# ChanghyeonKim93/visual_odometry_ros

Measured on AMD Instinct MI355X. Metric: stereo VO frames/sec @1241x376, 1500 feats, higher is better.
Workload: dtype u8/i32 (KLT, FAST) + f32 (IC, GN, DLT) + f64 (local BA)

## Files before the change

include/vo_hip.h:

```cpp
#ifndef VO_HIP_H_
#define VO_HIP_H_

#include <stddef.h>
#include <stdint.h>

#ifdef __cplusplus
extern "C" {
#endif

#define VO_HIP_ABI_VERSION 3

typedef enum {
  VO_OK = 0,
  VO_ERR_INVALID = -1,
  VO_ERR_HIP = -2,
  VO_ERR_NO_DEVICE = -3,
  VO_ERR_SIZE = -4,
  VO_ERR_NAN_AXAY = -5,
  VO_ERR_NAN_PATCH = -6,
  VO_ERR_NAN_UPDATE = -7,
  VO_ERR_CAPACITY = -8,
  VO_ERR_GN_FAILED = -9,
  VO_ERR_LBA_NAN = -10
} vo_status;

#define VO_KLT_USE_INITIAL_FLOW 4

#define VO_GN_VARIANT_CORE 0
#define VO_GN_VARIANT_STANDALONE 1

typedef struct vo_ctx vo_ctx;

typedef struct {
  int device;
  int max_width;
  int max_height;
  int max_points;
  int n_slots;
  int max_level;
} vo_config;

typedef struct {
  int iterations;
  float err;
  float delta_err;
  float delta_norm;
  int cnt_invalid;
  int is_nan;
} vo_gn_info;

int vo_abi_version(void);
int vo_device_count(void);
int vo_create(const vo_config *cfg, vo_ctx **out);
void vo_destroy(vo_ctx *ctx);
const char *vo_last_error(const vo_ctx *ctx);
void *vo_stream(vo_ctx *ctx);
int vo_synchronize(vo_ctx *ctx);

enum { VO_SUM_ORDER_TREE = 0, VO_SUM_ORDER_REFERENCE = 1 };
int vo_set_sum_order(vo_ctx *ctx, int order);
int vo_get_sum_order(const vo_ctx *ctx);

int vo_set_image(vo_ctx *ctx, int slot, const uint8_t *host, int width, int height, int stride);
int vo_set_image_device(vo_ctx *ctx, int slot, const void *dev, int width, int height, int stride);
int vo_swap_slots(vo_ctx *ctx, int slot_a, int slot_b);
int vo_set_stereo_pair_device(vo_ctx *ctx, int slot_l, const void *dev_l, int slot_r, const void *dev_r,
                              int width, int height, int stride);
int vo_set_ingest_side_stream(vo_ctx *ctx, int on);
int vo_set_stereo_pair_host_async(vo_ctx *ctx, int slot_l, const uint8_t *host_l, int slot_r, const uint8_t *host_r,
                                  int width, int height, int stride);
int vo_set_pyramid_window_hint(vo_ctx *ctx, int win);
int vo_pyramid_levels(int width, int height, int win, int max_level);
int vo_get_level(vo_ctx *ctx, int slot, int level, uint8_t *host, int *width, int *height);

int vo_klt_track(vo_ctx *ctx, int slot0, int slot1, const float *pts0, float *pts1, int n,
                 int win, int max_level, int flags, int max_iter, double eps, float min_eig_thr,
                 uint8_t *status, float *err);

int vo_track(vo_ctx *ctx, int slot0, int slot1, const float *pts0, int n, int win, int max_level,
             float thres_err, float *pts_track, uint8_t *mask_valid);
int vo_track_bidirection(vo_ctx *ctx, int slot0, int slot1, const float *pts0, int n, int win,
                         int max_level, float thres_err, float thres_bidirection,
                         float *pts_track, uint8_t *mask_valid);
int vo_track_bidirection_with_prior(vo_ctx *ctx, int slot0, int slot1, const float *pts0, int n,
                                    int win, int max_level, float thres_err,
                                    float thres_bidirection, float *pts_track,
                                    uint8_t *mask_valid);
int vo_track_with_prior(vo_ctx *ctx, int slot0, int slot1, const float *pts0, int n, int win,
                        int max_level, float thres_err, float *pts_track, uint8_t *mask_valid);
int vo_calc_prior(vo_ctx *ctx, const float *pts0, int n_pts0, const float *Xw, int n,
                  const float Tw1[16], const float K[9], float *pts1_prior);
int vo_track_with_scale(vo_ctx *ctx, int slot0, int slot1, const float *pts0,
                        const float *scale_est, int n, float *pts_track, uint8_t *mask_valid,
                        int strict_border);

int vo_gn_pose_mono(vo_ctx *ctx, const float *X, const float *pts1, int n, const float K[4],
                    int thres_reproj_outlier, float R01[9], float t01[3], uint8_t *mask_inlier,
                    int variant, vo_gn_info *info);
int vo_gn_pose_stereo(vo_ctx *ctx, const float *X, const float *pts_l1, const float *pts_r1,
                      int n, const float Kl[4], const float Kr[4], const float T_lr[16],
                      float thres_reproj_outlier, float T01[16], uint8_t *mask_inlier,
                      vo_gn_info *info);

int vo_gn_pose_information_stereo(vo_ctx *ctx, const float *X, const float *pts_l1, const float *pts_r1, int n,
                                  const float Kl[4], const float Kr[4], const float T_lr[16], const float T01[16],
                                  double sigma_px, double H[36], double Sigma[36], double *s2, int *valid);
int vo_gn_pose_information_mono(vo_ctx *ctx, const float *X, const float *pts1, int n, const float K[4],
                                const float R01[9], const float t01[3], double sigma_px, double H[36], double Sigma[36],
                                double *s2, int *valid);

int vo_se3_exp(vo_ctx *ctx, const float xi[6], float T[16], float Tinv[16]);

int vo_sampson_distance(vo_ctx *ctx, const float *pts0, const float *pts1, int n, const float F10[9],
                        float *dist);
int vo_symmetric_epipolar_distance(vo_ctx *ctx, const float *pts0, const float *pts1, int n,
                                   const float F10[9], float *dist);

int vo_weight_bin_update(vo_ctx *ctx, const float *pts, int n, int u_step, int v_step, int n_bins_u,
                         int n_bins_v, int32_t *weight);
int vo_bucket_argmax(vo_ctx *ctx, const float *kp_xy, const float *kp_response, int n, float inv_u_step,
                     float inv_v_step, int n_bins_u, int n_bins_v, const int32_t *weight, float *pts_out,
                     int32_t *idx_out, int *n_out);

typedef struct {
  int nfeatures;
  double scale_factor;
  int n_levels;
  int edge_threshold;
  int fast_threshold;
} vo_orb_params;
int vo_orb_detect(vo_ctx *ctx, int slot, const vo_orb_params *prm, float *kp_xy, float *kp_response,
                  int32_t *kp_octave, int max_kp, int *n_out);
int vo_orb_get_level(vo_ctx *ctx, int level, uint8_t *host, int *width, int *height);
int vo_extract_orb_with_binning(vo_ctx *ctx, int slot, const vo_orb_params *prm, float inv_u_step, float inv_v_step,
                                int n_bins_u, int n_bins_v, const int32_t *weight, float *pts_out, int *n_out,
                                int *n_detected);

int vo_extract_orb_with_binning_enqueue(vo_ctx *ctx, int slot, const vo_orb_params *prm, float inv_u_step,
                                        float inv_v_step, int n_bins_u, int n_bins_v, const int32_t *weight);
int vo_extract_orb_with_binning_result(vo_ctx *ctx, float *pts_out, int *n_out, int *n_detected);

int vo_orb_hamming(vo_ctx *ctx, const uint8_t *a, int na, const uint8_t *b, int nb,
                   uint16_t *dist);
int vo_orb_match(vo_ctx *ctx, const uint8_t *a, int na, const uint8_t *b, int nb, int th_low,
                 float ratio, int32_t *best_idx, uint16_t *best_dist, uint16_t *second_dist);

int vo_orb_default_pattern(int8_t pattern[1024]);
int vo_orb_get_pattern(vo_ctx *ctx, int8_t pattern[1024]);
int vo_orb_set_pattern(vo_ctx *ctx, const int8_t pattern[1024]);
int vo_orb_compute(vo_ctx *ctx, int slot, const vo_orb_params *prm, const float *kp_xy, const int32_t *kp_octave, int n,
                   int steer, float *angle_out, uint8_t *desc_out, uint8_t *valid_out);
int vo_orb_detect_and_compute(vo_ctx *ctx, int slot, const vo_orb_params *prm, int steer, int set, float *kp_xy,
                              float *kp_response, int32_t *kp_octave, float *kp_angle, uint8_t *desc, int max_kp, int *n_out);
int vo_orb_match_sets(vo_ctx *ctx, int set_a, int set_b, int th_low, float ratio, int32_t *best_idx, uint16_t *best_dist,
                      uint16_t *second_dist);

int vo_compact_indices(vo_ctx *ctx, const uint8_t *mask, const uint8_t *alive,
                       const uint8_t *tracked, int n, int32_t *index_valid, int *n_out);

int vo_ids_reset(vo_ctx *ctx, int32_t next_landmark_id, int32_t next_frame_id);
int vo_ids_peek(const vo_ctx *ctx, int32_t *next_landmark_id, int32_t *next_frame_id);
int vo_ids_new_frames(vo_ctx *ctx, int n, int32_t *ids);
int vo_ids_new_landmarks(vo_ctx *ctx, const uint8_t *accept, int n, int32_t *ids, int *n_created);
int vo_compact_tracks(vo_ctx *ctx, const uint8_t *mask, const uint8_t *alive, uint8_t *tracked, const int32_t *ids,
                      int n, int32_t *index_valid, int32_t *ids_out, int *n_out);

typedef struct {
  int width, height;
  int win, max_level;
  float thres_err, thres_bidirection, thres_poseba;
  float Kl[4], Kr[4];
  float T_lr[16];
  float thres_sampson;
} vo_stereo_params;

typedef struct {
  int n_l0l1, n_refine, n_l1r1, n_inlier, n_new_ok;
  int gn_iterations;
  int n_replayed;
  int n_ba;
} vo_frame_counts;

#define VO_LM_TRIANGULATED 1
#define VO_LM_DROPPED 2
#define VO_MONO_LM_BUNDLED 1
#define VO_MONO_LM_BA_CLASS 2
#define VO_MONO_LM_DROPPED 4

int vo_stereo_frame_set_strict_border(vo_ctx *ctx, int strict);

int vo_stereo_frame_recoveries(const vo_ctx *ctx);

enum { VO_DBG_FAIL_JOIN = 0, VO_DBG_CONC_GRID = 1, VO_DBG_SBA_LDS_SOLVE = 2, VO_DBG_SKIP_DETECT = 3, VO_OPT_POLL_YIELD = 4,
       VO_DBG_MVO_HOST_ADVANCE = 5, VO_DBG_STAGED_DETECT = 6, VO_DBG_CANDS_IN_FRAME = 7, VO_DBG_SBA_SPLIT = 8,
       VO_DBG_SDP_STAGE = 9, VO_DBG_SDW_FORM = 10, VO_DBG_COUNT = 11 };
int vo_debug_set(vo_ctx *ctx, int key, int value);
int vo_debug_allocation_count(const vo_ctx *ctx, long long *count);

int vo_stereo_frame_enqueue(vo_ctx *ctx, const vo_stereo_params *prm, int slot_l0, int slot_l1,
                            int slot_r1, const float *pts_l0, const float *pts_r0,
                            const float *Xp, const uint8_t *flags, int n, const float dT_prior[16],
                            const float *pts_new, int n_new, int inputs_on_device);
typedef struct {
  int n_bins_u, n_bins_v;
  int u_step, v_step;
  float inv_u_step, inv_v_step;
  vo_orb_params orb;
} vo_bin_params;
int vo_new_point_candidates_enqueue(vo_ctx *ctx, int slot, const vo_bin_params *bins, int table);
int vo_new_point_candidates_get(vo_ctx *ctx, int table, float *xy, uint8_t *has, int *n_detected);
int vo_stereo_frame_enqueue_closed(vo_ctx *ctx, const vo_stereo_params *prm, int slot_l0, int slot_l1, int slot_r1,
                                   const float *pts_l0, const float *pts_r0, const float *Xp, const uint8_t *flags,
                                   int n, const float dT_prior[16], const vo_bin_params *bins, int table,
                                   int inputs_on_device);
int vo_stereo_frame_enqueue_closed_world(vo_ctx *ctx, const vo_stereo_params *prm, int slot_l0, int slot_l1, int slot_r1,
                                         const float *pts_l0, const float *pts_r0, const float *Xw, const uint8_t *flags,
                                         int n, const float dT_prior[16], const float T_pw[16], const float T_cw_prior[16],
                                         const vo_bin_params *bins, int table, int inputs_on_device);
int vo_stereo_frame_new_points(vo_ctx *ctx, float *pts_new, int *n_new);

int vo_stereo_frame_result(vo_ctx *ctx, float *pts_l1, float *pts_r1, uint8_t *stage,
                           float dT[16], float *pts_new_r, uint8_t *mask_new,
                           vo_frame_counts *counts, vo_gn_info *gn);

typedef struct vo_svo vo_svo;
typedef struct {
  vo_stereo_params frame;
  vo_bin_params bins;
  float kf_overlap_ratio;
  float kf_rotation_deg;
  float kf_translation;
  int kf_window;
  int strict_border;
  int local_ba;
  int rectify;
} vo_svo_params;
typedef struct {
  int frame_id;
  int is_first, is_keyframe, lba_ran;
  int n_tracks_in;
  int n_final;
  int n_new;
  int n_tracks_out;
  int n_kf_tracked;
  int n_new_candidates;
  vo_frame_counts counts;
  vo_gn_info gn;
  float dT[16];
  float T_wc[16];
  double lba_err_first, lba_err_last;
  int lba_landmarks, lba_observations;
} vo_svo_frame_info;
int vo_svo_create(vo_ctx *ctx, const vo_svo_params *prm, vo_svo **out);
void vo_svo_destroy(vo_svo *svo);
int vo_svo_track(vo_svo *svo, const void *left, const void *right, int stride, int on_device, double timestamp,
                 vo_svo_frame_info *info);
int vo_svo_enqueue(vo_svo *svo, const void *left, const void *right, int stride, int on_device, double timestamp);
int vo_svo_prefetch(vo_svo *svo, const void *left, const void *right, int stride, int on_device);
int vo_svo_result(vo_svo *svo, vo_svo_frame_info *info);
int vo_svo_run(vo_svo *svo, const void *const *left, const void *const *right, int n_total, int stride, int on_device,
               int k_begin, int k_end, vo_svo_frame_info *infos, double *stamps);
#define VO_LM_KF_MEMBER 4
int vo_svo_get_tracks(vo_svo *svo, int32_t *ids, float *pts_l, float *pts_r, float *Xw, uint8_t *flags, int cap, int *n);
int vo_svo_get_new_points(vo_svo *svo, float *pts_l, float *pts_r, uint8_t *mask_new, uint8_t *accept, int *n);
int vo_triangulate_dlt(vo_ctx *ctx, const float *pts0, const float *pts1, int n, const float T_10[16], const float K0[4],
                       const float K1[4], float *X0, float *X1);

typedef struct vo_batch vo_batch;
int vo_batch_create(const vo_config *cfg, const vo_svo_params *prm, int n_streams, vo_batch **out);
void vo_batch_destroy(vo_batch *batch);
const char *vo_batch_last_error(const vo_batch *batch);
int vo_batch_debug_set(vo_batch *batch, int key, int value);
int vo_batch_strict_border(const vo_batch *batch);
int vo_batch_run(vo_batch *batch, const void *const *left, const void *const *right, int n_frames, int stride, int on_device,
                 int warmup, float *T_wc, int32_t *last_ids, int ids_cap, int *n_ids, double *seconds, double *wall);

int vo_svo_keyframe_count(vo_svo *svo, int *n_keyframes);
int vo_svo_get_keyframe(vo_svo *svo, int j, float T_wc[16], float *mappoints, int cap, int *n_points);
int vo_svo_get_keyframes(vo_svo *svo, float *T_wc, int32_t *n_points, float *mappoints, size_t cap_points, size_t *total_points);
int vo_svo_device_bytes(const vo_svo *svo, size_t *bytes);
int vo_svo_set_debug_image(vo_svo *svo, int on);
int vo_svo_get_debug_image(vo_svo *svo, uint8_t *out, int out_stride, int *width, int *height);
int vo_svo_set_pose_covariance(vo_svo *svo, int on, double sigma_px);
int vo_svo_get_pose_covariance(vo_svo *svo, double P[36], double Sigma_xi[36], double *s2, int *valid, int *n_points,
                               int *n_unknown_steps);
int vo_svo_get_pose_covariance_inputs(vo_svo *svo, float *X, float *pts_l, float *pts_r, int cap, int *n, float T01[16]);

int vo_set_slot_mask(vo_ctx *ctx, int slot, const void *mask, int stride, int on_device);
int vo_slot_image_size(vo_ctx *ctx, int slot, int *width, int *height);
int vo_svo_set_mask(vo_svo *svo, const void *mask, int stride, int on_device);

enum { VO_ZNCC_PATTERN_REFERENCE = 0, VO_ZNCC_PATTERN_CENTERED = 1 };
enum { VO_ZNCC_TEMPORAL = 1, VO_ZNCC_STEREO = 2 };
int vo_zncc(vo_ctx *ctx, int slot0, int slot1, const float *pts0, const float *pts1, int n, int win, int pattern, float *out);
int vo_svo_set_zncc_gate(vo_svo *svo, int pairs, int win, int pattern, float thres);
int vo_svo_get_zncc(vo_svo *svo, float *zncc_t, float *zncc_s, int cap, int *n);

typedef struct {
  int hw, hh;
  int d_min, d_max;
  int g_min;
  float thres_best;
  float thres_peak;
  int peak_px;
  int edge_px;
  float eps_edge;
  float eps_epi;
  float bf;
} vo_semidense_params;
enum { VO_SEMIDENSE_KEYFRAMES = 0, VO_SEMIDENSE_FRAMES = 1 };
int vo_semidense_default_params(vo_semidense_params *prm);
int vo_semidense_stereo(vo_ctx *ctx, int slot_l, int slot_r, const vo_semidense_params *prm, float *disparity, float *score,
                        float *sigma_invd, uint8_t *status, int on_device);
int vo_semidense_points(vo_ctx *ctx, const float *disparity, const float *sigma_invd, const uint8_t *status, int width, int height,
                        int planes_on_device, const float K[4], float bf, const float *T, int cap, float *xyz, float *sigma_out,
                        uint16_t *pixel, int *n);
int vo_svo_set_semidense(vo_svo *svo, const vo_semidense_params *prm, int every);
int vo_svo_get_semidense(vo_svo *svo, float *disparity, float *score, float *sigma_invd, uint8_t *status, int *width, int *height,
                         int *frame_id, float T_wc[16], int *n_accepted);
int vo_svo_get_semidense_points(vo_svo *svo, int world, int cap, float *xyz, float *sigma_invd, uint16_t *pixel, int *n, int *frame_id);

typedef struct {
  int d_min;
  int n_disp;
  int paths;
  int p1, p2;
  int uniqueness;
  int lr_max;
  float eps_d;
  float bf;
} vo_dense_stereo_params;
int vo_dense_stereo_default_params(vo_dense_stereo_params *prm);
int vo_dense_stereo_workspace(int width, int height, const vo_dense_stereo_params *prm, size_t *bytes);
int vo_dense_stereo(vo_ctx *ctx, int slot_l, int slot_r, const vo_dense_stereo_params *prm, float *disparity, uint16_t *cost,
                    float *sigma_invd, uint8_t *status, int on_device);
int vo_svo_set_dense_stereo(vo_svo *svo, const vo_dense_stereo_params *prm, int every);
int vo_svo_get_dense_stereo(vo_svo *svo, float *disparity, uint16_t *cost, float *sigma_invd, uint8_t *status, int *width, int *height,
                            int *frame_id, float T_wc[16], int *n_accepted);
int vo_svo_get_dense_points(vo_svo *svo, int world, int cap, float *xyz, float *sigma_invd, uint16_t *pixel, int *n, int *frame_id);

#define VO_DISPARITY_SPECKLE 6
typedef struct {
  int max_size;
  float max_diff;
} vo_speckle_params;
int vo_speckle_default_params(vo_speckle_params *prm);
int vo_speckle_workspace(int width, int height, size_t *bytes);
int vo_disparity_speckle_filter(vo_ctx *ctx, float *disparity, float *sigma_invd, uint8_t *status, int width, int height,
                                const vo_speckle_params *prm, int32_t *label, int32_t *size, int *n_removed, int *n_components,
                                int on_device);
int vo_svo_set_dense_speckle(vo_svo *svo, const vo_speckle_params *prm);
int vo_svo_get_dense_speckle_stats(vo_svo *svo, int *n_removed, int *n_components);

typedef struct {
  float chi;
  int keep_obs;
} vo_semidense_map_merge_params;
int vo_semidense_map_merge_default_params(vo_semidense_map_merge_params *prm);
int vo_semidense_map_merge(vo_ctx *ctx, const float *map_invd, const float *map_sigma, const uint8_t *map_n_obs, const float *disparity,
                           const float *sigma_invd, const uint8_t *status, int width, int height, float bf,
                           const vo_semidense_map_merge_params *prm, float *invd, float *sigma, uint8_t *n_obs, uint8_t *origin,
                           uint64_t *counts, int on_device);
int vo_svo_set_semidense_world_merge(vo_svo *svo, const vo_semidense_map_merge_params *prm);
int vo_svo_get_semidense_world_source(vo_svo *svo, float *invd, float *sigma, uint8_t *n_obs, uint8_t *origin, int *width, int *height,
                                      int *frame_id, uint64_t *counts);

typedef struct {
  int hw, hh;
  int g_min;
  float thres_best;
  float thres_peak;
  int peak_px;
  int edge_px;
  float eps_edge;
  float eps_epi;
  float eps_scale;
  float z_min, z_max;
  int max_search;
  float j_min;
} vo_semidense_temporal_params;
int vo_semidense_temporal_default_params(vo_semidense_temporal_params *prm);
int vo_semidense_map_seed(vo_ctx *ctx, const float *disparity, const float *sigma_invd, const uint8_t *status, int width, int height,
                          float bf, float *invd, float *sigma, uint8_t *n_obs, uint8_t *tstatus, int on_device);
int vo_semidense_temporal(vo_ctx *ctx, const uint8_t *key_plane, int key_stride, int key_on_device, int slot_cur, const float K[4],
                          const float T_ck[16], const vo_semidense_temporal_params *prm, float *invd, float *sigma, uint8_t *n_obs,
                          uint8_t *tstatus, float *score, int on_device);
int vo_semidense_map_points(vo_ctx *ctx, const float *invd, const float *sigma, const uint8_t *n_obs, int width, int height,
                            int planes_on_device, const float K[4], const float *T, int min_obs, int cap, float *xyz, float *sigma_out,
                            uint16_t *pixel, int *n);
int vo_svo_set_semidense_temporal(vo_svo *svo, const vo_semidense_temporal_params *prm);
int vo_svo_get_semidense_map(vo_svo *svo, float *invd, float *sigma, uint8_t *n_obs, uint8_t *tstatus, int *width, int *height,
                             int *frame_id, float T_wc[16], int *n_fused);
int vo_svo_get_semidense_map_points(vo_svo *svo, int world, int min_obs, int cap, float *xyz, float *sigma, uint16_t *pixel, int *n,
                                    int *frame_id);

typedef struct {
  int min_obs;
  int max_diff;
  float chi;
  float sigma_add;
} vo_semidense_propagate_params;
int vo_semidense_propagate_default_params(vo_semidense_propagate_params *prm);
int vo_semidense_map_propagate(vo_ctx *ctx, const float *old_invd, const float *old_sigma, const uint8_t *old_n_obs, const uint8_t *key_plane,
                               int key_stride, int slot_new, const float *disparity, const float *sigma_invd, const uint8_t *status, float bf,
                               const float K[4], const float T_ba[16], const vo_semidense_propagate_params *prm, float *invd, float *sigma,
                               uint8_t *n_obs, uint8_t *tstatus, uint8_t *origin, int32_t *src, int on_device);
int vo_svo_set_semidense_propagate(vo_svo *svo, const vo_semidense_propagate_params *prm);
int vo_svo_get_semidense_origin(vo_svo *svo, uint8_t *origin, int *width, int *height, int *from_frame_id);

enum { VO_SEMIDENSE_ALIGN_CONVERGED = 0, VO_SEMIDENSE_ALIGN_MAX_ITERS = 1, VO_SEMIDENSE_ALIGN_FEW_PIXELS = 2, VO_SEMIDENSE_ALIGN_SINGULAR = 3,
       VO_SEMIDENSE_ALIGN_NONE = 4 };
typedef struct {
  int min_obs;
  float huber;
  int max_iters;
  float eps;
  int min_pixels;
} vo_semidense_align_params;
typedef struct {
  float T_ck[16];
  int status, iters, count;
  double rms;
  double H[21], b[6];
} vo_semidense_align_result;
int vo_semidense_align_default_params(vo_semidense_align_params *prm);
int vo_semidense_align(vo_ctx *ctx, const uint8_t *key_plane, int key_stride, int key_on_device, int slot_cur, const float K[4],
                       const float T_ck[16], const vo_semidense_align_params *prm, const float *invd, const float *sigma, const uint8_t *n_obs,
                       int on_device, vo_semidense_align_result *result);
int vo_svo_set_semidense_align(vo_svo *svo, const vo_semidense_align_params *prm);
int vo_svo_get_semidense_align(vo_svo *svo, vo_semidense_align_result *result, float T_wc[16], int *frame_id, int *key_frame_id);

#define VO_SEMIDENSE_ALIGN_MAX_LEVELS 6
enum { VO_SEMIDENSE_ALIGN_START_ODOMETRY = 0, VO_SEMIDENSE_ALIGN_START_PREVIOUS = 1 };
typedef struct {
  int min_obs;
  float huber;
  int max_iters;
  float eps;
  int min_pixels;
  int levels;
  int max_iters_level[VO_SEMIDENSE_ALIGN_MAX_LEVELS];
} vo_semidense_align_pyr_params;
typedef struct {
  float T_ck[16];
  int status, iters, count;
  double rms;
  double H[21], b[6];
  int levels, start_prev;
  int level_status[VO_SEMIDENSE_ALIGN_MAX_LEVELS], level_iters[VO_SEMIDENSE_ALIGN_MAX_LEVELS], level_count[VO_SEMIDENSE_ALIGN_MAX_LEVELS];
  double level_rms[VO_SEMIDENSE_ALIGN_MAX_LEVELS];
} vo_semidense_align_pyr_result;
int vo_semidense_align_pyr_default_params(vo_semidense_align_pyr_params *prm);
int vo_semidense_map_pyramid_size(int width, int height, int levels, long long *elements);
int vo_semidense_map_pyramid(vo_ctx *ctx, const float *invd, const float *sigma, const uint8_t *n_obs, int width, int height, int levels,
                             float *invd_pyr, float *sigma_pyr, uint8_t *n_obs_pyr, int on_device);
int vo_semidense_align_pyr(vo_ctx *ctx, int slot_key, int slot_cur, const float K[4], const float T_ck[16],
                           const vo_semidense_align_pyr_params *prm, const float *invd, const float *sigma, const uint8_t *n_obs, int on_device,
                           vo_semidense_align_pyr_result *result);
int vo_svo_set_semidense_align_pyr(vo_svo *svo, const vo_semidense_align_pyr_params *prm, int start);
int vo_svo_get_semidense_align_pyr(vo_svo *svo, vo_semidense_align_pyr_result *result, float T_wc[16], int *frame_id, int *key_frame_id);

enum { VO_SEMIDENSE_ALIGN_AFFINE_RANGE = 5 };
typedef struct {
  float gain0;
  float offset0;
} vo_semidense_affine_params;
typedef struct {
  float T_ck[16];
  int status, iters, count;
  double rms;
  double H[36], b[8];
  double gain, offset;
  int G, O;
  int levels, start_prev;
  int level_status[VO_SEMIDENSE_ALIGN_MAX_LEVELS], level_iters[VO_SEMIDENSE_ALIGN_MAX_LEVELS], level_count[VO_SEMIDENSE_ALIGN_MAX_LEVELS];
  double level_rms[VO_SEMIDENSE_ALIGN_MAX_LEVELS];
  int level_G[VO_SEMIDENSE_ALIGN_MAX_LEVELS], level_O[VO_SEMIDENSE_ALIGN_MAX_LEVELS];
} vo_semidense_align_affine_result;
int vo_semidense_affine_default_params(vo_semidense_affine_params *prm);
int vo_semidense_align_affine(vo_ctx *ctx, const uint8_t *key_plane, int key_stride, int key_on_device, int slot_cur, const float K[4],
                              const float T_ck[16], const vo_semidense_align_params *prm, const vo_semidense_affine_params *affine,
                              const float *invd, const float *sigma, const uint8_t *n_obs, int on_device,
                              vo_semidense_align_affine_result *result);
int vo_semidense_align_pyr_affine(vo_ctx *ctx, int slot_key, int slot_cur, const float K[4], const float T_ck[16],
                                  const vo_semidense_align_pyr_params *prm, const vo_semidense_affine_params *affine, const float *invd,
                                  const float *sigma, const uint8_t *n_obs, int on_device, vo_semidense_align_affine_result *result);
int vo_svo_set_semidense_align_affine(vo_svo *svo, const vo_semidense_affine_params *affine);
int vo_svo_get_semidense_align_affine(vo_svo *svo, vo_semidense_align_affine_result *result, float T_wc[16], int *frame_id, int *key_frame_id);

typedef struct {
  int radius;
  float chi;
  float dist_sigma;
  int min_support;
  int fill_min;
  int g_min;
} vo_semidense_regularize_params;
int vo_semidense_regularize_default_params(vo_semidense_regularize_params *prm);
// ... 230 lines not shown
```

visual_odometry_ros_amd/api.py:

```python
import collections
import ctypes as C
import os
import weakref

import numpy as np

from . import _capi
from ._capi import (FIVE_POINT_FN, BinParams, FivePointInfo, FivePointParams, FrameCounts, GnInfo, MonoCounts, MonoParams, MvoFrameInfo, MvoParams, OrbParams,
                    SbaProblem, StereoParams, SvoFrameInfo, SvoParams, VoConfig, VoError)

KLT_USE_INITIAL_FLOW = 4
GN_CORE, GN_STANDALONE = 0, 1


def _f32(a):
    return np.ascontiguousarray(a, dtype=np.float32)


def _u8(a):
    return np.ascontiguousarray(a, dtype=np.uint8)


def _p(a, t=C.c_float):
    return a.ctypes.data_as(C.POINTER(t))
# ... 173 lines not shown

class SemiDenseMerged(collections.namedtuple("SemiDenseMerged", "invd sigma n_obs origin counts frame_id", defaults=(None,))):
    __slots__ = ()


def _semidense_merge_params(lib, params):
    p = _capi.SemiDenseMapMergeParams()
    lib.vo_semidense_map_merge_default_params(C.byref(p))
    known = {f[0] for f in _capi.SemiDenseMapMergeParams._fields_}
    for k, v in ({} if params is True else dict(params)).items():
        if k not in known:
            raise ValueError(f"semi-dense map merge: unknown parameter {k!r}; known: {sorted(known)}")
        setattr(p, k, v)
    return p


class SemiDenseWorldPoints(collections.namedtuple("SemiDenseWorldPoints", "index xyz weight count keyframes grey sums", defaults=(None,))):
    __slots__ = ()


class SemiDenseWorldFreePoints(collections.namedtuple("SemiDenseWorldFreePoints", "index xyz weight count keyframes grey sums free")):
    __slots__ = ()


def _semidense_world_params(lib, params):
    p = _capi.SemiDenseWorldParams()
    lib.vo_semidense_world_default_params(C.byref(p))
    known = {f[0] for f in _capi.SemiDenseWorldParams._fields_}
    for k, v in dict(params).items():
        if k not in known:
            raise ValueError(f"semi-dense world map: unknown parameter {k!r}; known: {sorted(known)}")
        setattr(p, k, v)
    return p


def _semidense_world_carve_params(lib, params):
    p = _capi.SemiDenseWorldCarveParams()
    lib.vo_semidense_world_carve_default_params(C.byref(p))
    known = {f[0] for f in _capi.SemiDenseWorldCarveParams._fields_}
    for k, v in ({} if params is True else dict(params)).items():
        if k not in known:
            raise ValueError(f"world map carving: unknown parameter {k!r}; known: {sorted(known)}")
        setattr(p, k, v)
    return p


def _max_free(max_free):
    num, den = (int(v) for v in max_free)
    return num, den


def _semidense_world_points(check, get, capacity, with_sums, with_free=False):
    n = C.c_int()
    if capacity is None:
        rc = get(0, None, None, None, None, None, None, *((None,) if with_sums else ()), *((None,) if with_free else ()), C.byref(n))
        if rc < 0 and rc != -8:
            check(rc)
        capacity = n.value
    cap = int(capacity)
    m = max(cap, 1)
    idx, xyz = np.zeros((m, 3), np.int32), np.zeros((m, 3), np.float32)
    wt, cnt, kf, grey = np.zeros(m, np.uint32), np.zeros(m, np.uint32), np.zeros(m, np.uint32), np.zeros(m, np.uint8)
    sums, free = np.zeros((m, 5), np.uint64), np.zeros(m, np.uint32)
    rc = get(cap, idx.ctypes.data, xyz.ctypes.data, wt.ctypes.data, cnt.ctypes.data, kf.ctypes.data, grey.ctypes.data,
             *((sums.ctypes.data,) if with_sums else ()), *((free.ctypes.data,) if with_free else ()), C.byref(n))
    try:
        check(rc)
    except VoError as e:
        e.n = n.value
        raise
    k = min(n.value, cap)
    if with_free:
        return SemiDenseWorldFreePoints(idx[:k], xyz[:k], wt[:k], cnt[:k], kf[:k], grey[:k], sums[:k] if with_sums else None, free[:k])
    return SemiDenseWorldPoints(idx[:k], xyz[:k], wt[:k], cnt[:k], kf[:k], grey[:k], sums[:k] if with_sums else None)


class SemiDenseWorld:

    def __init__(self, ctx, **params):
        self.ctx, self.lib = ctx, ctx.lib
        self.params = _semidense_world_params(self.lib, params)
        self._h = C.c_void_p()
        ctx.check(self.lib.vo_semidense_world_create(ctx.handle, C.byref(self.params), C.byref(self._h)))
        ctx._children.add(self)

    def integrate(self, map, K, T_wk, key=None, on_device=None, key_on_device=None):
        self._launch(self.lib.vo_semidense_world_integrate, map, K, (T_wk,), key, on_device, key_on_device)

    def remove(self, map, K, T_wk, key=None, on_device=None, key_on_device=None):
        self._launch(self.lib.vo_semidense_world_remove, map, K, (T_wk,), key, on_device, key_on_device)

    def reanchor(self, map, K, T_old, T_new, key=None, on_device=None, key_on_device=None):
        moved = C.c_int()
        self._launch(self.lib.vo_semidense_world_reanchor, map, K, (T_old, T_new), key, on_device, key_on_device, C.byref(moved))
        return bool(moved.value)

    def carve(self, map, K, T_wk, on_device=None, **params):
        p = _semidense_world_carve_params(self.lib, params)
        get = (lambda k: getattr(map, k)) if isinstance(map, tuple) else (lambda k: map[k])
        Ka = np.ascontiguousarray(K, np.float32).reshape(4)
        T = np.ascontiguousarray(T_wk, np.float32).reshape(4, 4)
        if on_device is not None:
            w, h = on_device
            planes = [C.c_void_p(get(k)) for k in ("invd", "sigma", "n_obs")]
        else:
            invd, sigma = np.ascontiguousarray(get("invd"), np.float32), np.ascontiguousarray(get("sigma"), np.float32)
            n_obs = np.ascontiguousarray(get("n_obs"), np.uint8)
            if invd.ndim != 2 or sigma.shape != invd.shape or n_obs.shape != invd.shape:
                raise ValueError("invd, sigma and n_obs are planes of one (height, width)")
            h, w = invd.shape
            planes = [invd.ctypes.data, sigma.ctypes.data, n_obs.ctypes.data]
        self.ctx.check(self.lib.vo_semidense_world_carve(self._h, *planes, int(w), int(h), int(on_device is not None), Ka.ctypes.data,
                                                         T.ctypes.data, C.byref(p)))

    def carveStats(self):
        info = _capi.SemiDenseWorldCarveInfo()
        self.ctx.check(self.lib.vo_semidense_world_carve_stats(self._h, C.byref(info)))
        return {k: int(getattr(info, k)) for k, _ in _capi.SemiDenseWorldCarveInfo._fields_}

    def reanchorStats(self):
        info = _capi.SemiDenseWorldReanchorInfo()
        self.ctx.check(self.lib.vo_semidense_world_reanchor_stats(self._h, C.byref(info)))
        return {k: int(getattr(info, k)) for k, _ in _capi.SemiDenseWorldReanchorInfo._fields_}

    def _launch(self, fn, map, K, poses, key, on_device, key_on_device, *tail):
        get = (lambda k: getattr(map, k)) if isinstance(map, tuple) else (lambda k: map[k])
        Ka = np.ascontiguousarray(K, np.float32).reshape(4)
        Ts = [np.ascontiguousarray(T, np.float32).reshape(4, 4) for T in poses]
        if on_device is not None:
            w, h = on_device
            planes = [C.c_void_p(get(k)) for k in ("invd", "sigma", "n_obs")]
        else:
            invd, sigma = np.ascontiguousarray(get("invd"), np.float32), np.ascontiguousarray(get("sigma"), np.float32)
            n_obs = np.ascontiguousarray(get("n_obs"), np.uint8)
            if invd.ndim != 2 or sigma.shape != invd.shape or n_obs.shape != invd.shape:
                raise ValueError("invd, sigma and n_obs are planes of one (height, width)")
            h, w = invd.shape
            planes = [invd.ctypes.data, sigma.ctypes.data, n_obs.ctypes.data]
        if key is None:
            pk, stride = None, 0
        elif key_on_device is not None:
            pk, stride = C.c_void_p(key), int(key_on_device)
        else:
            ka = _u8(key)
            if ka.shape != (h, w):
                raise ValueError("key is a plane of the map's (height, width)")
            pk, stride = ka.ctypes.data, ka.strides[0]
        self.ctx.check(fn(self._h, *planes, pk, stride, int(key_on_device is not None), int(w), int(h), int(on_device is not None),
                          Ka.ctypes.data, *(T.ctypes.data for T in Ts), *tail))

    def points(self, min_count=1, min_keyframes=1, capacity=None, max_free=None):
        if max_free is not None:
            num, den = _max_free(max_free)
            get = lambda cap, *a: self.lib.vo_semidense_world_points_free(self._h, int(min_count), int(min_keyframes), num, den, cap, *a)
            return _semidense_world_points(self.ctx.check, get, capacity, True, True)
        get = lambda *a: self.lib.vo_semidense_world_points(self._h, int(min_count), int(min_keyframes), *a)
        return _semidense_world_points(self.ctx.check, get, capacity, True)

    def stats(self):
        info = _capi.SemiDenseWorldInfo()
        self.ctx.check(self.lib.vo_semidense_world_stats(self._h, C.byref(info)))
        return {k: int(getattr(info, k)) for k, _ in _capi.SemiDenseWorldInfo._fields_}

    def clear(self):
        self.ctx.check(self.lib.vo_semidense_world_clear(self._h))

    def close(self):
        if self._h:
            self.lib.vo_semidense_world_destroy(self._h)
            self._h = C.c_void_p()

    def __enter__(self):
        return self

    def __exit__(self, *a):
        self.close()


SEMIDENSE_ALIGN_STATUS = {0: "converged", 1: "max_iters reached", 2: "too few pixels", 3: "singular system", 4: "no result"}


SEMIDENSE_ALIGN_START = {"odometry": 0, "previous": 1}
SemiDenseAlignedLevel = collections.namedtuple("SemiDenseAlignedLevel", "status iters count rms")
SEMIDENSE_ALIGN_AFFINE_STATUS = {**SEMIDENSE_ALIGN_STATUS, 5: "gain or offset left its range"}
SemiDenseAlignedAffineLevel = collections.namedtuple("SemiDenseAlignedAffineLevel", "status iters count rms G O")


class SemiDenseAligned(collections.namedtuple("SemiDenseAligned",
                                              "T_ck status iters count rms H b T_wc frame_id key_frame_id levels start gain offset G O",
                                              defaults=(None, None, None, None, None, None))):
    __slots__ = ()


def _semidense_align_params(lib, params):
    p = _capi.SemiDenseAlignParams()
    lib.vo_semidense_align_default_params(C.byref(p))
    known = {f[0] for f in _capi.SemiDenseAlignParams._fields_}
    for k, v in dict(params).items():
        if k not in known:
            raise ValueError(f"semi-dense alignment: unknown parameter {k!r}; known: {sorted(known)}")
        setattr(p, k, v)
    return p


def _semidense_align_pyr_params(lib, params):
    p = _capi.SemiDenseAlignPyrParams()
    lib.vo_semidense_align_pyr_default_params(C.byref(p))
    known = {f[0] for f in _capi.SemiDenseAlignPyrParams._fields_}
    for k, v in dict(params).items():
        if k not in known:
            raise ValueError(f"semi-dense alignment: unknown parameter {k!r}; known: {sorted(known)}")
        if k == "max_iters_level":
            v = [int(x) for x in v]
            if len(v) > 6:
                raise ValueError("semi-dense alignment: max_iters_level holds at most 6 counts")
            v = (C.c_int * 6)(*(v + [0] * (6 - len(v))))
        setattr(p, k, v)
    return p


def _semidense_affine_params(lib, affine):
    p = _capi.SemiDenseAffineParams()
    lib.vo_semidense_affine_default_params(C.byref(p))
    known = {f[0] for f in _capi.SemiDenseAffineParams._fields_}
    for k, v in ({} if affine is True else dict(affine)).items():
        if k not in known:
            raise ValueError(f"semi-dense alignment, affine brightness: unknown parameter {k!r}; known: {sorted(known)}")
        setattr(p, k, v)
    return p


def _semidense_aligned(r, T_wc=None, frame_id=None, key_frame_id=None, with_levels=True):
    affine = isinstance(r, _capi.SemiDenseAlignAffineResult)
    nu = 8 if affine else 6
    H = np.zeros((nu, nu), np.float64)
    n = 0
    for i in range(nu):
        for j in range(i, nu):
            H[i, j] = H[j, i] = r.H[n]
            n += 1
    levels = start = None
    if affine:
        if with_levels:
            levels = tuple(SemiDenseAlignedAffineLevel(int(r.level_status[l]), int(r.level_iters[l]), int(r.level_count[l]),
                                                       float(r.level_rms[l]), int(r.level_G[l]), int(r.level_O[l])) for l in range(r.levels))
        start = None if frame_id is None else ("previous" if r.start_prev else "odometry")
        return SemiDenseAligned(np.array(r.T_ck, np.float32).reshape(4, 4), int(r.status), int(r.iters), int(r.count), float(r.rms), H,
                                np.array(r.b, np.float64), T_wc, frame_id, key_frame_id, levels, start, float(r.gain), float(r.offset),
                                int(r.G), int(r.O))
    if isinstance(r, _capi.SemiDenseAlignPyrResult):
        levels = tuple(SemiDenseAlignedLevel(int(r.level_status[l]), int(r.level_iters[l]), int(r.level_count[l]), float(r.level_rms[l]))
                       for l in range(r.levels))
        start = None if frame_id is None else ("previous" if r.start_prev else "odometry")
    return SemiDenseAligned(np.array(r.T_ck, np.float32).reshape(4, 4), int(r.status), int(r.iters), int(r.count), float(r.rms), H,
                            np.array(r.b, np.float64), T_wc, frame_id, key_frame_id, levels, start)


def _zncc_gate_arg(gate, stereo):
    if gate is None:
        return 0, 15, 1, 0.0
    if not isinstance(gate, dict) or "thres" not in gate or not set(gate) <= {"thres", "win", "pattern", "pairs"}:
        raise ValueError(f"zncc_gate must be None or dict(thres=, win=, pattern=, pairs=), not {gate!r}")
    pattern = gate.get("pattern", "centered")
    if pattern not in Context.ZNCC_PATTERNS:
        raise ValueError(f"pattern must be one of {sorted(Context.ZNCC_PATTERNS)}, not {pattern!r}")
    pairs = gate.get("pairs", ("temporal",))
    if isinstance(pairs, str):
        pairs = (pairs,)
    bits = 0
    for p in pairs:
        if p not in Context.ZNCC_PAIRS or (p == "stereo" and not stereo):
            raise ValueError(f'pairs must be out of {"temporal, stereo" if stereo else "temporal"}, not {p!r}')
        bits |= Context.ZNCC_PAIRS[p]
    if not bits:
        raise ValueError("pairs is empty: pass None to switch the gate off")
    return bits, int(gate.get("win", 15)), Context.ZNCC_PATTERNS[pattern], float(gate["thres"])


class Context:

    SUM_ORDERS = {"tree": 0, "reference": 1}

    def __init__(self, device=0, max_width=1241, max_height=376, max_points=4096, n_slots=4,
                 max_level=6, sum_order="tree"):
        if sum_order not in self.SUM_ORDERS:
            raise ValueError(f"sum_order must be one of {sorted(self.SUM_ORDERS)}, not {sum_order!r}")
        self.lib = _capi.load()
        self._h = C.c_void_p()
        cfg = VoConfig(device, max_width, max_height, max_points, n_slots, max_level)
        rc = self.lib.vo_create(C.byref(cfg), C.byref(self._h))
        if rc != 0:
            msg = self.lib.vo_last_error(self._h if self._h else None).decode()
            if self._h:
                self.lib.vo_destroy(self._h)
                self._h = C.c_void_p()
            raise VoError(rc, msg)
        self.cfg = cfg
        self.sum_order = sum_order
        self._children = weakref.WeakSet()
        self.debug_switches = {}
        if os.environ.get("VO_TEST_SWITCHES") == "1":
            for key, name in ((0, "VO_DEBUG_FAIL_JOIN"), (1, "VO_CONC_GRID"), (2, "VO_SBA_LDS_SOLVE"), (3, "VO_DEBUG_SKIP_DETECT"),
                              (5, "VO_MVO_HOST_ADVANCE"), (6, "VO_STAGED_DETECT"), (7, "VO_CANDS_IN_FRAME"),
                              (8, "VO_SBA_SPLIT")):
                v = os.environ.get(name)
                if v:
                    self.debug_set(key, int(v) if v.lstrip("-").isdigit() else 1)
                    self.debug_switches[name] = v

    DBG_FAIL_JOIN, DBG_CONC_GRID, DBG_SBA_LDS_SOLVE, DBG_SKIP_DETECT, OPT_POLL_YIELD, DBG_MVO_HOST_ADVANCE, DBG_STAGED_DETECT, DBG_CANDS_IN_FRAME = 0, 1, 2, 3, 4, 5, 6, 7
    DBG_SBA_SPLIT = 8
    DBG_SDP_STAGE = 9

    @property
    def sum_order(self):
        order = self.lib.vo_get_sum_order(self._h)
        self.check(order)
        return {v: k for k, v in self.SUM_ORDERS.items()}[order]

    @sum_order.setter
    def sum_order(self, order):
        if order not in self.SUM_ORDERS:
            raise ValueError(f"sum_order must be one of {sorted(self.SUM_ORDERS)}, not {order!r}")
        self.check(self.lib.vo_set_sum_order(self._h, self.SUM_ORDERS[order]))

    def debug_set(self, key, value):
        self.check(self.lib.vo_debug_set(self._h, int(key), int(value)))

    def allocation_count(self):
        n = C.c_longlong(0)
        self.check(self.lib.vo_debug_allocation_count(self._h, C.byref(n)))
        return n.value

    def close(self):
        if getattr(self, "_h", None):
            for ch in list(getattr(self, "_children", ())):
                ch.close()
            self.lib.vo_destroy(self._h)
            self._h = C.c_void_p()

    def __del__(self):
        try:
            self.close()
        except Exception:
            pass

    def __enter__(self):
        return self

    def __exit__(self, *a):
        self.close()

    def check(self, rc):
        if rc < 0:
            raise VoError(rc, self.lib.vo_last_error(self._h).decode())
        return rc

    @property
    def handle(self):
        return self._h

    @property
    def stream(self):
        return self.lib.vo_stream(self._h)

    def synchronize(self):
        self.check(self.lib.vo_synchronize(self._h))

    def set_image(self, slot, img):
        img = _u8(img)
        assert img.ndim == 2
        self.check(self.lib.vo_set_image(self._h, slot, _p(img, C.c_uint8), img.shape[1], img.shape[0],
                                         img.strides[0]))

    def slot_image_size(self, slot):
        w, h = C.c_int(), C.c_int()
        self.check(self.lib.vo_slot_image_size(self._h, slot, C.byref(w), C.byref(h)))
        return w.value, h.value

    def set_slot_mask(self, slot, mask):
        w, h = self.slot_image_size(slot) if mask is not None else (0, 0)
        if mask is not None and w == 0:
            raise VoError(-1, f"slot {slot} holds no image: a mask has the dimensions of the slot's image")
        _, ptr, stride, dev = _mask_arg(mask, w, h)
        self.check(self.lib.vo_set_slot_mask(self._h, slot, ptr, stride, dev))

    ZNCC_PATTERNS = {"reference": 0, "centered": 1}
    ZNCC_PAIRS = {"temporal": 1, "stereo": 2}

    def calcZNCC(self, slot0, slot1, pts0, pts1, win=15, pattern="reference"):
        if pattern not in self.ZNCC_PATTERNS:
            raise ValueError(f"pattern must be one of {sorted(self.ZNCC_PATTERNS)}, not {pattern!r}")
        p0 = np.ascontiguousarray(pts0, np.float32).reshape(-1, 2)
        p1 = np.ascontiguousarray(pts1, np.float32).reshape(-1, 2)
        if len(p0) != len(p1):
            raise ValueError("pts0 and pts1 must hold the same number of points")
        out = np.zeros(len(p0), np.float32)
        self.check(self.lib.vo_zncc(self._h, int(slot0), int(slot1), p0.ctypes.data, p1.ctypes.data, len(p0), int(win),
                                    self.ZNCC_PATTERNS[pattern], out.ctypes.data))
        return out

    def semiDenseStereo(self, slot_l, slot_r, out=None, **params):
        p = _semidense_params(self.lib, params)
        if out is not None:
            ptr = [C.c_void_p(out.get(k)) if out.get(k) else None for k in ("disparity", "score", "sigma_invd", "status")]
            self.check(self.lib.vo_semidense_stereo(self._h, int(slot_l), int(slot_r), C.byref(p), *ptr, 1))
            return None
        w, h = self.slot_image_size(slot_l)
        if w <= 0:
            raise VoError(-1, f"slot {slot_l} holds no image")
        d, sc, sg = (np.zeros((h, w), np.float32) for _ in range(3))
        st = np.zeros((h, w), np.uint8)
        self.check(self.lib.vo_semidense_stereo(self._h, int(slot_l), int(slot_r), C.byref(p), d.ctypes.data, sc.ctypes.data, sg.ctypes.data,
                                                st.ctypes.data, 0))
        return SemiDenseResult(d, sc, sg, st, None, None, int((st == 1).sum()))

    def denseStereo(self, slot_l, slot_r, out=None, speckle=None, **params):
        p = _dense_stereo_params(self.lib, params)
        sp = None if speckle is None or speckle is False else _speckle_params(self.lib, speckle)
        if out is not None:
            if sp is not None and not (out.get("disparity") and out.get("status")):
                raise ValueError("denseStereo: speckle needs the disparity and status planes in out")
            ptr = [C.c_void_p(out.get(k)) if out.get(k) else None for k in ("disparity", "cost", "sigma_invd", "status")]
            self.check(self.lib.vo_dense_stereo(self._h, int(slot_l), int(slot_r), C.byref(p), *ptr, 1))
            if sp is not None:
                w, h = self.slot_image_size(slot_l)
                self.check(self.lib.vo_disparity_speckle_filter(self._h, ptr[0], ptr[2], ptr[3], w, h, C.byref(sp), None, None, None, None, 1))
            return None
        w, h = self.slot_image_size(slot_l)
        if w <= 0:
            raise VoError(-1, f"slot {slot_l} holds no image")
        d, sg = (np.zeros((h, w), np.float32) for _ in range(2))
        co, st = np.zeros((h, w), np.uint16), np.zeros((h, w), np.uint8)
        self.check(self.lib.vo_dense_stereo(self._h, int(slot_l), int(slot_r), C.byref(p), d.ctypes.data, co.ctypes.data, sg.ctypes.data,
                                            st.ctypes.data, 0))
        if sp is not None:
            self.check(self.lib.vo_disparity_speckle_filter(self._h, d.ctypes.data, sg.ctypes.data, st.ctypes.data, w, h, C.byref(sp), None, None,
                                                            None, None, 0))
        return DenseStereoResult(d, co, sg, st, None, None, int((st == 1).sum()))

    def disparitySpeckleFilter(self, disparity, sigma_invd, status, max_size=100, max_diff=1.0, labels=False, on_device=None):
        p = _speckle_params(self.lib, dict(max_size=max_size, max_diff=max_diff))
        nr, nc = C.c_int(), C.c_int()
        if on_device is not None:
            w, h = on_device
            lab = labels if isinstance(labels, dict) else {}
            self.check(self.lib.vo_disparity_speckle_filter(self._h, C.c_void_p(disparity), C.c_void_p(sigma_invd) if sigma_invd else None,
                                                            C.c_void_p(status), int(w), int(h), C.byref(p),
                                                            C.c_void_p(lab["label"]) if lab.get("label") else None,
                                                            C.c_void_p(lab["size"]) if lab.get("size") else None, C.byref(nr), C.byref(nc), 1))
            return SpeckleResult(None, None, None, None, None, nr.value, nc.value)
        d, st = np.array(disparity, np.float32, order="C"), np.array(status, np.uint8, order="C")
        sg = None if sigma_invd is None else np.array(sigma_invd, np.float32, order="C")
        if d.ndim != 2 or st.shape != d.shape or (sg is not None and sg.shape != d.shape):
            raise ValueError("disparity, sigma_invd and status are planes of one (height, width)")
        lab, sz = (np.zeros(d.shape, np.int32) for _ in range(2)) if labels else (None, None)
        self.check(self.lib.vo_disparity_speckle_filter(self._h, d.ctypes.data, None if sg is None else sg.ctypes.data, st.ctypes.data, d.shape[1],
                                                        d.shape[0], C.byref(p), None if lab is None else lab.ctypes.data,
                                                        None if sz is None else sz.ctypes.data, C.byref(nr), C.byref(nc), 0))
        return SpeckleResult(d, sg, st, lab, sz, nr.value, nc.value)

    def disparitySpeckleWorkspace(self, width, height):
        n = C.c_size_t()
        self.check(self.lib.vo_speckle_workspace(int(width), int(height), C.byref(n)))
        return n.value

    def denseStereoWorkspace(self, width, height, **params):
        p = _dense_stereo_params(self.lib, params)
        n = C.c_size_t()
        self.check(self.lib.vo_dense_stereo_workspace(int(width), int(height), C.byref(p), C.byref(n)))
        return n.value

    def semiDensePoints(self, disparity, sigma_invd, status, K, bf, T=None, capacity=None, on_device=None):
        if on_device is not None:
            w, h = on_device
            pd, ps, pt = C.c_void_p(disparity), C.c_void_p(sigma_invd), C.c_void_p(status)
        else:
            d = np.ascontiguousarray(disparity, np.float32)
            sg = np.ascontiguousarray(sigma_invd, np.float32)
            st = np.ascontiguousarray(status, np.uint8)
            if d.ndim != 2 or sg.shape != d.shape or st.shape != d.shape:
                raise ValueError("disparity, sigma_invd and status are planes of one (height, width)")
            h, w = d.shape
            pd, ps, pt = d.ctypes.data, sg.ctypes.data, st.ctypes.data
        cap = w * h if capacity is None else int(capacity)
        Ka = np.ascontiguousarray(K, np.float32).reshape(4)
        Ta = None if T is None else np.ascontiguousarray(T, np.float32).reshape(4, 4)
        xyz, so, px = np.zeros((max(cap, 1), 3), np.float32), np.zeros(max(cap, 1), np.float32), np.zeros((max(cap, 1), 2), np.uint16)
        n = C.c_int()
        rc = self.lib.vo_semidense_points(self._h, pd, ps, pt, w, h, int(on_device is not None), Ka.ctypes.data, float(bf),
                                          None if Ta is None else Ta.ctypes.data, cap, xyz.ctypes.data, so.ctypes.data, px.ctypes.data, C.byref(n))
        try:
            self.check(rc)
        except VoError as e:
            e.n = n.value
            raise
        return xyz[:n.value], so[:n.value], px[:n.value]

    def semiDenseMapSeed(self, disparity, sigma_invd, status, bf, out=None, on_device=None):
        if on_device is not None:
            w, h = on_device
            self.check(self.lib.vo_semidense_map_seed(self._h, C.c_void_p(disparity), C.c_void_p(sigma_invd), C.c_void_p(status), int(w), int(h),
                                                      float(bf), *(C.c_void_p(out[k]) for k in ("invd", "sigma", "n_obs", "tstatus")), 1))
            return None
        d, sg, st = np.ascontiguousarray(disparity, np.float32), np.ascontiguousarray(sigma_invd, np.float32), np.ascontiguousarray(status, np.uint8)
        if d.ndim != 2 or sg.shape != d.shape or st.shape != d.shape:
            raise ValueError("disparity, sigma_invd and status are planes of one (height, width)")
        invd, sigma = np.zeros(d.shape, np.float32), np.zeros(d.shape, np.float32)
        n_obs, ts = np.zeros(d.shape, np.uint8), np.zeros(d.shape, np.uint8)
        self.check(self.lib.vo_semidense_map_seed(self._h, d.ctypes.data, sg.ctypes.data, st.ctypes.data, d.shape[1], d.shape[0], float(bf),
                                                  invd.ctypes.data, sigma.ctypes.data, n_obs.ctypes.data, ts.ctypes.data, 0))
        return SemiDenseMap(invd, sigma, n_obs, ts, None, None, None, None)

    def semiDenseMapMerge(self, map, dense, bf, chi=3.0, keep_obs=2, out=None, on_device=None):
        p = _semidense_merge_params(self.lib, dict(chi=chi, keep_obs=keep_obs))
        getm = None if map is None else ((lambda k: getattr(map, k)) if isinstance(map, tuple) and hasattr(map, "_fields") else (lambda k: map[k]))
        if hasattr(dense, "_fields"):
            dp = [getattr(dense, k) for k in ("disparity", "sigma_invd", "status")]
        elif isinstance(dense, dict):
            dp = [dense[k] for k in ("disparity", "sigma_invd", "status")]
        else:
            dp = list(dense)
            if len(dp) != 3:
                raise ValueError("semiDenseMapMerge: dense is a result or its planes disparity, sigma_invd, status")
        counts = np.zeros(6, np.uint64)
        if on_device is not None:
            w, h = on_device
            mp = [None] * 3 if map is None else [C.c_void_p(getm(k)) for k in ("invd", "sigma", "n_obs")]
            self.check(self.lib.vo_semidense_map_merge(self._h, *mp, *(C.c_void_p(x) for x in dp), int(w), int(h), float(bf), C.byref(p),
                                                       *(C.c_void_p(out[k]) for k in ("invd", "sigma", "n_obs")),
                                                       C.c_void_p(out["origin"]) if out.get("origin") else None, counts.ctypes.data, 1))
            return SemiDenseMerged(None, None, None, None, counts)
        d, sg, st = np.ascontiguousarray(dp[0], np.float32), np.ascontiguousarray(dp[1], np.float32), np.ascontiguousarray(dp[2], np.uint8)
        if d.ndim != 2 or sg.shape != d.shape or st.shape != d.shape:
            raise ValueError("disparity, sigma_invd and status are planes of one (height, width)")
        mp = [None] * 3
        if map is not None:
            keep = [np.ascontiguousarray(getm("invd"), np.float32), np.ascontiguousarray(getm("sigma"), np.float32),
                    np.ascontiguousarray(getm("n_obs"), np.uint8)]
            if any(x.shape != d.shape for x in keep):
                raise ValueError("the map's planes and the result's are of one (height, width)")
            mp = [x.ctypes.data for x in keep]
        invd, sigma = np.zeros(d.shape, np.float32), np.zeros(d.shape, np.float32)
        n_obs, origin = np.zeros(d.shape, np.uint8), np.zeros(d.shape, np.uint8)
        self.check(self.lib.vo_semidense_map_merge(self._h, *mp, d.ctypes.data, sg.ctypes.data, st.ctypes.data, d.shape[1], d.shape[0], float(bf),
                                                   C.byref(p), invd.ctypes.data, sigma.ctypes.data, n_obs.ctypes.data, origin.ctypes.data,
                                                   counts.ctypes.data, 0))
        return SemiDenseMerged(invd, sigma, n_obs, origin, counts)

    def semiDenseTemporal(self, key, slot_cur, K, T_ck, map, key_on_device=None, map_on_device=False, **params):
        p = _semidense_temporal_params(self.lib, params)
        Ka = np.ascontiguousarray(K, np.float32).reshape(4)
        Ta = np.ascontiguousarray(T_ck, np.float32).reshape(4, 4)
        if key_on_device is not None:
            pk, stride = C.c_void_p(key), int(key_on_device)
        else:
            ka = _u8(key)
            pk, stride = ka.ctypes.data, ka.strides[0]
        if map_on_device:
            sc = map.get("score")
            self.check(self.lib.vo_semidense_temporal(self._h, pk, stride, int(key_on_device is not None), int(slot_cur), Ka.ctypes.data, Ta.ctypes.data,
                                                      C.byref(p), *(C.c_void_p(map[k]) for k in ("invd", "sigma", "n_obs", "tstatus")),
                                                      C.c_void_p(sc) if sc else None, 1))
            return None
        get = (lambda k: getattr(map, k)) if isinstance(map, SemiDenseMap) else (lambda k: map[k])
        invd, sigma = np.array(get("invd"), np.float32, order="C"), np.array(get("sigma"), np.float32, order="C")
        n_obs = np.array(get("n_obs"), np.uint8, order="C")
        w, h = self.slot_image_size(slot_cur)
        if invd.shape != (h, w) or sigma.shape != (h, w) or n_obs.shape != (h, w):
            raise ValueError(f"the map's planes must be ({h}, {w}) like slot {slot_cur}'s image")
        ts, score = np.zeros((h, w), np.uint8), np.zeros((h, w), np.float32)
        self.check(self.lib.vo_semidense_temporal(self._h, pk, stride, int(key_on_device is not None), int(slot_cur), Ka.ctypes.data, Ta.ctypes.data,
                                                  C.byref(p), invd.ctypes.data, sigma.ctypes.data, n_obs.ctypes.data, ts.ctypes.data, score.ctypes.data, 0))
        return SemiDenseMap(invd, sigma, n_obs, ts, score, None, None, None)

    def semiDenseAlign(self, key, slot_cur, K, T_ck, map, key_on_device=None, map_on_device=False, affine=None, **params):
        p = _semidense_align_params(self.lib, params)
        Ka = np.ascontiguousarray(K, np.float32).reshape(4)
        Ta = np.ascontiguousarray(T_ck, np.float32).reshape(4, 4)
        if key_on_device is not None:
            pk, stride = C.c_void_p(key), int(key_on_device)
        else:
            ka = _u8(key)
            pk, stride = ka.ctypes.data, ka.strides[0]
        get = (lambda k: getattr(map, k)) if isinstance(map, tuple) else (lambda k: map[k])
        res = _capi.SemiDenseAlignResult()
        if map_on_device:
            planes = [C.c_void_p(get(k)) for k in ("invd", "sigma", "n_obs")]
        else:
            invd, sigma = np.ascontiguousarray(get("invd"), np.float32), np.ascontiguousarray(get("sigma"), np.float32)
            n_obs = np.ascontiguousarray(get("n_obs"), np.uint8)
            w, h = self.slot_image_size(slot_cur)
            if invd.shape != (h, w) or sigma.shape != (h, w) or n_obs.shape != (h, w):
                raise ValueError(f"the map's planes must be ({h}, {w}) like slot {slot_cur}'s image")
            planes = [invd.ctypes.data, sigma.ctypes.data, n_obs.ctypes.data]
        if affine:
            ap, res = _semidense_affine_params(self.lib, affine), _capi.SemiDenseAlignAffineResult()
            self.check(self.lib.vo_semidense_align_affine(self._h, pk, stride, int(key_on_device is not None), int(slot_cur), Ka.ctypes.data,
                                                          Ta.ctypes.data, C.byref(p), C.byref(ap), *planes, int(bool(map_on_device)), C.byref(res)))
            return _semidense_aligned(res, with_levels=False)
        self.check(self.lib.vo_semidense_align(self._h, pk, stride, int(key_on_device is not None), int(slot_cur), Ka.ctypes.data, Ta.ctypes.data,
                                               C.byref(p), *planes, int(bool(map_on_device)), C.byref(res)))
        return _semidense_aligned(res)

    def semiDenseMapPyramid(self, map, levels, on_device=None, out=None):
        get = (lambda k: getattr(map, k)) if isinstance(map, tuple) else (lambda k: map[k])
        if on_device is not None:
            w, h = on_device
            self.check(self.lib.vo_semidense_map_pyramid(self._h, *(C.c_void_p(get(k)) for k in ("invd", "sigma", "n_obs")), int(w), int(h),
                                                         int(levels), *(C.c_void_p(out[k]) for k in ("invd", "sigma", "n_obs")), 1))
            return None
        invd, sigma = np.ascontiguousarray(get("invd"), np.float32), np.ascontiguousarray(get("sigma"), np.float32)
        n_obs = np.ascontiguousarray(get("n_obs"), np.uint8)
        if invd.ndim != 2 or sigma.shape != invd.shape or n_obs.shape != invd.shape:
            raise ValueError("invd, sigma and n_obs are planes of one (height, width)")
# ... 2163 lines not shown
```

visual_odometry_ros_amd/csrc/stereo_vo_lba.hip:

```cpp
#include <math.h>
#include <sched.h>
#include <stdint.h>
#include <stdlib.h>
#include <time.h>

#include <algorithm>

#include "sba_device.hpp"
#include "stereo_vo.hpp"

static double lba_now() {
  timespec ts;
  clock_gettime(CLOCK_MONOTONIC, &ts);
  return 1e6 * (double)ts.tv_sec + 1e-3 * (double)ts.tv_nsec;
}

static void mul44d(const double A[16], const double B[16], double C[16]) {
  double R[16];
  for (int i = 0; i < 4; ++i)
    for (int j = 0; j < 4; ++j) {
      double r = A[i * 4 + 0] * B[0 * 4 + j];
      for (int k = 1; k < 4; ++k) r = A[i * 4 + k] * B[k * 4 + j] + r;
      R[i * 4 + j] = r;
    }
  for (int i = 0; i < 16; ++i) C[i] = R[i];
}
static void inv_se3d(const double T[16], double Ti[16]) {
  double Rt[9];
  for (int i = 0; i < 3; ++i)
    for (int j = 0; j < 3; ++j) Rt[i * 3 + j] = T[j * 4 + i];
  const double t[3] = {T[3], T[7], T[11]};
  for (int i = 0; i < 3; ++i) {
    for (int j = 0; j < 3; ++j) Ti[i * 4 + j] = Rt[i * 3 + j];
    Ti[i * 4 + 3] = (-Rt[i * 3 + 0]) * t[0] + ((-Rt[i * 3 + 1]) * t[1] + (-Rt[i * 3 + 2]) * t[2]);
  }
  Ti[12] = Ti[13] = Ti[14] = 0.0;
  Ti[15] = 1.0;
}
static void to_d(const float T[16], double D[16]) {
  for (int i = 0; i < 12; ++i) D[i] = (double)T[i];
  D[12] = D[13] = D[14] = 0.0;
  D[15] = 1.0;
}

#define LBA_KW 16
#define LBA_TAB_FIRST_BITS 18
#define LBA_TAB_BITS 24
#define LBA_SPAN_MAX (1 << LBA_TAB_BITS)
#define LBA_SPAN_FIRST (1 << 16)

struct LmTab {
  float *X;
  uint8_t *S;
  int32_t *tag;
  int mask;
};
struct LbaWin {
  int nk, No, W, base;
  int kw;
  int opk;
  int n[LBA_KW];
  const int32_t *ids[LBA_KW];
  const float *pl[LBA_KW], *pr[LBA_KW];
  int opt[LBA_KW];
  int optf[LBA_KW];
  int optmask;
};
struct LbaProb {
  double *T, *X, *px;
  int *opt_index, *opt_frame, *obs_ptr, *obs_frame, *slot_ptr, *slot_j, *slot_bobs, *slot_lm;
  uint8_t *obs_right;
  int *pose_obs_ptr, *pose_obs_end, *pose_obs, *pose_lm, *pose_slot_ptr, *pose_slot_end, *pose_slot;
  int *pair_ptr, *pair_end, *pair_a, *pair_b;
  int *flags, *dyn;
  double *avg_err;
  int32_t *used_id;
  int *lm_mask;
  int *mask_w, *q_w;
  unsigned long long *pre, *wg_tot;
  int pose_obs_stride, pose_slot_stride, pair_stride, max_iter;
};

__global__ void lba_keyframe_kernel(SvoTrackSet ts, int n, LmTab tab, int32_t *kf_ids, float *kf_pl, float *kf_pr, int32_t *all_ids) {
  const int k = blockIdx.x * blockDim.x + threadIdx.x;
  if (k >= n) return;
  const int32_t id = ts.ids[k];
  const int t = id & tab.mask;
  const uint8_t dead = tab.tag[t] == id ? (uint8_t)(tab.S[t] & 2) : (uint8_t)0;
  tab.X[3 * (size_t)t] = ts.Xw[3 * k];
  tab.X[3 * (size_t)t + 1] = ts.Xw[3 * k + 1];
  tab.X[3 * (size_t)t + 2] = ts.Xw[3 * k + 2];
  tab.S[t] = (uint8_t)(dead | ((ts.flags[k] & VO_LM_TRIANGULATED) ? 1 : 0) | ((ts.flags[k] & VO_LM_BUNDLED) ? 4 : 0));
  tab.tag[t] = id;
  kf_ids[k] = id;
  all_ids[k] = id;
  kf_pl[2 * k] = ts.pts_l[2 * k];
  kf_pl[2 * k + 1] = ts.pts_l[2 * k + 1];
  kf_pr[2 * k] = ts.pts_r[2 * k];
  kf_pr[2 * k + 1] = ts.pts_r[2 * k + 1];
}

__global__ void lba_table_update_kernel(SvoTrackSet ts, int n, LmTab tab) {
  const int k = blockIdx.x * blockDim.x + threadIdx.x;
  if (k >= n) return;
  const int32_t id = ts.ids[k];
  const int t = id & tab.mask;
  if (tab.tag[t] != id) return;
  tab.X[3 * (size_t)t] = ts.Xw[3 * k];
  tab.X[3 * (size_t)t + 1] = ts.Xw[3 * k + 1];
  tab.X[3 * (size_t)t + 2] = ts.Xw[3 * k + 2];
  tab.S[t] = (uint8_t)((tab.S[t] & 2) | ((ts.flags[k] & VO_LM_TRIANGULATED) ? 1 : 0) | ((ts.flags[k] & VO_LM_BUNDLED) ? 4 : 0));
}

__global__ void lba_scatter_kernel(LbaWin w, int *mask_w, int *q_w) {
  const int j = blockIdx.y, q = blockIdx.x * blockDim.x + threadIdx.x;
  if (q >= w.n[j]) return;
  const int idx = w.ids[j][q] - w.base;
  if ((unsigned)idx >= (unsigned)w.W) return;
  atomicOr(&mask_w[idx], 1 << j);
  q_w[(size_t)idx * w.kw + j] = q;
}

__device__ __forceinline__ int lba_block_scan(int v, int *s_w, int &total) {
  const int tid = threadIdx.x, lane = tid & 63, wave = tid >> 6;
  int inc = v;
#pragma unroll
  for (int off = 1; off < 64; off <<= 1) {
    const int t = __shfl_up(inc, off);
    if (lane >= off) inc += t;
  }
  __syncthreads();
  if (lane == 63) s_w[wave] = inc;
  __syncthreads();
  int before = 0, tot = 0;
#pragma unroll
  for (int k = 0; k < 16; ++k) {
    const int c = s_w[k];
    before += k < wave ? c : 0;
    tot += c;
  }
  total = tot;
  return before + inc - v;
}

template <int NW>
__device__ __forceinline__ unsigned long long lba_block_scan64(unsigned long long v, unsigned long long *s_w,
                                                               unsigned long long &total) {
  const int tid = threadIdx.x, lane = tid & 63, wave = tid >> 6;
  unsigned long long inc = v;
#pragma unroll
  for (int off = 1; off < 64; off <<= 1) {
    const unsigned long long t = __shfl_up(inc, off);
    if (lane >= off) inc += t;
  }
  __syncthreads();
  if (lane == 63) s_w[wave] = inc;
  __syncthreads();
  unsigned long long before = 0, tot = 0;
#pragma unroll
  for (int k = 0; k < NW; ++k) {
    const unsigned long long c = s_w[k];
    before += k < wave ? c : 0;
    tot += c;
  }
  total = tot;
  return before + inc - v;
}
#define LBA_PK_KF 20
#define LBA_PK_SL 42
#define LBA_QWG 256

__global__ __launch_bounds__(LBA_QWG) void lba_qualify_kernel(LbaWin w, LmTab tab, LbaProb p) {
  __shared__ unsigned long long s_w[LBA_QWG / 64];
  const int idx = blockIdx.x * LBA_QWG + threadIdx.x;
  int m = idx < w.W ? p.mask_w[idx] : 0;
  if (m) {
    const int32_t id = w.base + idx;
    const int t = id & tab.mask;
    const uint8_t st = tab.tag[t] == id ? tab.S[t] : (uint8_t)0;
    if (!((st & 1) && !(st & 2)) || w.opk * __popc(m) < 2) {
      m = 0;
      p.mask_w[idx] = 0;
    }
  }
  const unsigned long long v =
      m ? 1ull | ((unsigned long long)__popc(m) << LBA_PK_KF) | ((unsigned long long)__popc(m & w.optmask) << LBA_PK_SL) : 0ull;
  unsigned long long total;
  const unsigned long long ex = lba_block_scan64<LBA_QWG / 64>(v, s_w, total);
  if (idx < w.W) p.pre[idx] = ex;
  if (threadIdx.x == 0) p.wg_tot[blockIdx.x] = total;
}

struct LbaHead {
  double T_jw[16 * LBA_KW];
};
__global__ __launch_bounds__(1024) void lba_scan_kernel(LbaWin w, LbaProb p, LbaHead h, int n_wg) {
  __shared__ unsigned long long s_w[16];
  const int tid = threadIdx.x;
  for (int k = tid; k < 16 * w.nk; k += 1024) p.T[k] = h.T_jw[k];
  if (tid < w.nk) p.opt_index[tid] = w.opt[tid];
  if (tid < w.No) p.opt_frame[tid] = w.optf[tid];
  if (tid < 16) p.flags[tid] = 0;
  if (tid <= p.max_iter) p.avg_err[tid] = 0.0;
  const int chunk = (n_wg + 1023) / 1024, i0 = tid * chunk, i1 = min(i0 + chunk, n_wg);
  unsigned long long c = 0;
  for (int g = i0; g < i1; ++g) c += p.wg_tot[g];
  unsigned long long total, off = lba_block_scan64<16>(c, s_w, total);
  for (int g = i0; g < i1; ++g) {
    const unsigned long long t = p.wg_tot[g];
    p.wg_tot[g] = off;
    off += t;
  }
  if (tid == 0) {
    const int t_lm = (int)(total & ((1ull << LBA_PK_KF) - 1)), t_kf = (int)((total >> LBA_PK_KF) & ((1ull << (LBA_PK_SL - LBA_PK_KF)) - 1));
    const int t_sl = (int)(total >> LBA_PK_SL);
    p.dyn[0] = t_lm;
    p.dyn[1] = w.opk * t_kf;
    p.dyn[2] = t_sl;
    p.obs_ptr[t_lm] = w.opk * t_kf;
    p.slot_ptr[t_lm] = t_sl;
  }
}

struct LbaRef {
  double Tjw_ref[16], Twj_ref[16], inv_scale, pose_scale;
};
__global__ void lba_fill_kernel(LbaWin w, LmTab tab, LbaProb p, LbaRef r) {
  const int idx = blockIdx.x * blockDim.x + threadIdx.x;
  if (idx >= w.W) return;
  const int m = p.mask_w[idx];
  if (!m) return;
  p.mask_w[idx] = 0;
  const unsigned long long pk = p.pre[idx] + p.wg_tot[idx / LBA_QWG];
  const int i = (int)(pk & ((1ull << LBA_PK_KF) - 1)), kf0 = (int)((pk >> LBA_PK_KF) & ((1ull << (LBA_PK_SL - LBA_PK_KF)) - 1));
  const int s0 = (int)(pk >> LBA_PK_SL);
  const int32_t id = w.base + idx;
  const int t = id & tab.mask;
  p.used_id[i] = id;
  p.lm_mask[i] = m;
  const double Xd[3] = {(double)tab.X[3 * (size_t)t], (double)tab.X[3 * (size_t)t + 1], (double)tab.X[3 * (size_t)t + 2]};
#pragma unroll
  for (int k = 0; k < 3; ++k) {
    const double xr = (r.Tjw_ref[k * 4 + 0] * Xd[0] + (r.Tjw_ref[k * 4 + 1] * Xd[1] + r.Tjw_ref[k * 4 + 2] * Xd[2])) + r.Tjw_ref[k * 4 + 3];
    p.X[3 * (size_t)i + k] = xr * r.inv_scale;
  }
  p.obs_ptr[i] = w.opk * kf0;
  p.slot_ptr[i] = s0;
  int rr = 0, rs = 0;
  for (int mm = m; mm; mm &= mm - 1) {
    const int j = __ffs(mm) - 1;
    const int q = p.q_w[(size_t)idx * w.kw + j];
    const int o = w.opk * (kf0 + rr);
    p.obs_frame[o] = j;
    p.obs_right[o] = 0;
    p.px[2 * (size_t)o] = (double)w.pl[j][2 * q];
    p.px[2 * (size_t)o + 1] = (double)w.pl[j][2 * q + 1];
    if (w.opk == 2) {
      p.obs_frame[o + 1] = j;
      p.obs_right[o + 1] = 1;
      p.px[2 * (size_t)o + 2] = (double)w.pr[j][2 * q];
      p.px[2 * (size_t)o + 3] = (double)w.pr[j][2 * q + 1];
    }
    if (w.opt[j] >= 0) {
      const int s = s0 + rs;
      p.slot_j[s] = w.opt[j];
      p.slot_bobs[s] = o + w.opk - 1;
      p.slot_lm[s] = i;
      ++rs;
    }
    ++rr;
  }
}

__global__ __launch_bounds__(1024) void lba_lists_kernel(LbaWin w, LbaProb p) {
  __shared__ int s_w[16];
  const int tid = threadIdx.x, M = p.dyn[0], No = w.No;
  const int chunk = (M + 1023) / 1024, i0 = tid * chunk, i1 = min(i0 + chunk, M);
  int u = blockIdx.x;
  if (u < No) {
    const int f = w.optf[u], bit = 1 << f;
    int cnt = 0;
    for (int i = i0; i < i1; ++i) cnt += (p.lm_mask[i] & bit) ? 1 : 0;
    int total, off = lba_block_scan(cnt, s_w, total);
    const int Bo = u * p.pose_obs_stride, Bs = u * p.pose_slot_stride;
    for (int i = i0; i < i1; ++i) {
      const int m = p.lm_mask[i];
      if (!(m & bit)) continue;
      const int o = p.obs_ptr[i] + w.opk * __popc(m & (bit - 1));
      for (int e = 0; e < w.opk; ++e) {
        p.pose_obs[Bo + w.opk * off + e] = o + e;
        p.pose_lm[Bo + w.opk * off + e] = i;
      }
      p.pose_slot[Bs + off] = p.slot_ptr[i] + __popc(m & w.optmask & (bit - 1));
      ++off;
    }
    if (tid == 0) {
      p.pose_obs_ptr[u] = Bo;
      p.pose_obs_end[u] = Bo + w.opk * total;
      p.pose_slot_ptr[u] = Bs;
      p.pose_slot_end[u] = Bs + total;
    }
    return;
  }
  u -= No;
  int a = 0;
  while (u >= No - a) {
    u -= No - a;
    ++a;
  }
  const int b = a + u, jk = a * No + b;
  const int ba = 1 << w.optf[a], bb = 1 << w.optf[b], both = ba | bb;
  int cnt = 0;
  for (int i = i0; i < i1; ++i) cnt += ((p.lm_mask[i] & both) == both) ? 1 : 0;
  int total, off = lba_block_scan(cnt, s_w, total);
  const int Bp = jk * p.pair_stride;
  for (int i = i0; i < i1; ++i) {
    const int m = p.lm_mask[i];
    if ((m & both) != both) continue;
    const int sp = p.slot_ptr[i];
    p.pair_a[Bp + off] = sp + __popc(m & w.optmask & (ba - 1));
    p.pair_b[Bp + off] = sp + __popc(m & w.optmask & (bb - 1));
    ++off;
  }
  if (tid == 0) {
    p.pair_ptr[jk] = Bp;
    p.pair_end[jk] = Bp + total;
  }
}

__global__ void lba_writeback_kernel(LbaProb p, LmTab tab, LbaRef r) {
  const int i = blockIdx.x * blockDim.x + threadIdx.x;
  if (i >= p.dyn[0]) return;
  const double xs[3] = {p.X[3 * (size_t)i] * r.pose_scale, p.X[3 * (size_t)i + 1] * r.pose_scale, p.X[3 * (size_t)i + 2] * r.pose_scale};
  float L[3];
#pragma unroll
  for (int k = 0; k < 3; ++k)
    L[k] = (float)((r.Twj_ref[k * 4 + 0] * xs[0] + (r.Twj_ref[k * 4 + 1] * xs[1] + r.Twj_ref[k * 4 + 2] * xs[2])) + r.Twj_ref[k * 4 + 3]);
  const int t = p.used_id[i] & tab.mask;
  tab.X[3 * (size_t)t] = L[0];
  tab.X[3 * (size_t)t + 1] = L[1];
  tab.X[3 * (size_t)t + 2] = L[2];
  uint8_t st = (uint8_t)(tab.S[t] | 1);
  const float nrm = sqrtf(L[0] * L[0] + (L[1] * L[1] + L[2] * L[2]));
  if (!(nrm <= 3000))
    st |= 2;
  else
    st |= 4;
  tab.S[t] = st;
}
__global__ void lba_refresh_kernel(SvoTrackSet ts, int n, LmTab tab, int mono) {
  const int k = blockIdx.x * blockDim.x + threadIdx.x;
  if (k >= n) return;
  const int t = ts.ids[k] & tab.mask;
  ts.Xw[3 * k] = tab.X[3 * (size_t)t];
  ts.Xw[3 * k + 1] = tab.X[3 * (size_t)t + 1];
  ts.Xw[3 * k + 2] = tab.X[3 * (size_t)t + 2];
  uint8_t fl = ts.flags[k];
  const uint8_t st = tab.S[t];
  if (st & 1) fl |= VO_LM_TRIANGULATED;
  if (st & 2) fl |= VO_LM_DROPPED;
  if (mono && (st & 4)) fl |= VO_LM_BUNDLED;
  ts.flags[k] = fl;
}

__global__ void lba_mappoints_kernel(const int32_t *ids, int n, LmTab tab, float *out) {
  const int k = blockIdx.x * blockDim.x + threadIdx.x;
  if (k >= n) return;
  const int32_t id = ids[k];
  const int t = id & tab.mask;
  const bool ok = tab.tag[t] == id;
  out[3 * k] = ok ? tab.X[3 * (size_t)t] : 0.0f;
  out[3 * k + 1] = ok ? tab.X[3 * (size_t)t + 1] : 0.0f;
  out[3 * k + 2] = ok ? tab.X[3 * (size_t)t + 2] : 0.0f;
}

#define LBA_SEQ_WORD 1000
__global__ __launch_bounds__(256) void lba_result_kernel(const uint32_t *src, uint32_t *host, int words, uint32_t seq) {
  for (int k = threadIdx.x; k < words; k += 256) host[k] = src[k];
  __threadfence_system();
  __syncthreads();
  if (threadIdx.x == 0) __hip_atomic_store(&host[LBA_SEQ_WORD], seq, __ATOMIC_RELEASE, __HIP_MEMORY_SCOPE_SYSTEM);
}

__global__ void lba_tab_rehash_kernel(LmTab o, LmTab n) {
  const int t = blockIdx.x * blockDim.x + threadIdx.x;
  if (t > o.mask) return;
  const int32_t id = o.tag[t];
  if (id == -1) return;
  const int u = id & n.mask;
  n.X[3 * (size_t)u] = o.X[3 * (size_t)t];
  n.X[3 * (size_t)u + 1] = o.X[3 * (size_t)t + 1];
  n.X[3 * (size_t)u + 2] = o.X[3 * (size_t)t + 2];
  n.S[u] = o.S[t];
  n.tag[u] = id;
}

#define LBA_POOL_CHUNK ((size_t)1 << 20)
namespace {
struct Arena {
  size_t off = 0;
  size_t take(size_t bytes) {
    const size_t o = off;
    off += (bytes + 255) & ~(size_t)255;
    return o;
  }
};
struct LbaLayout {
  size_t res_bytes, oT, oAvg, oFl, oDyn, oOpt, oOfr, oX, oOp, oOf, oOr, oPx, oSp, oSj, oSb, oSl, oPop, oPo, oPl, oPsp, oPs, oPp,
      oPa, oPb, oUid, oLm, in_end, total;
  size_t E_max, Eopt_max;
  int No_max, maxn, n_err_max;
};
}

struct vo_svo_lba {
  LmTab tab = {};
  int tab_bits = 0;
  long long id_lo = 0;
  bool id_seen = false;
  int32_t *kf_ids[LBA_KW] = {};
  float *kf_pl[LBA_KW] = {}, *kf_pr[LBA_KW] = {};
  int *mask_w = nullptr, *q_w = nullptr;
  unsigned long long *pre = nullptr;
  size_t span_cap = 0;
  uint8_t *arena = nullptr;
  LbaLayout lay = {};
  uint8_t *h_res = nullptr;
  uint32_t seq = 0;
  std::vector<int32_t *> pool;
  size_t pool_used = 0;
  float *d_map = nullptr;
  float *d_map_all = nullptr;
  size_t map_all_cap = 0;
  std::vector<size_t> pool_fill;
  double tt[4] = {0, 0, 0, 0};
  int n_calls = 0;
};

void vo_svo_lba_free(vo_svo *s) {
  vo_svo_lba *L = s->lba;
  if (!L) return;
  void *dev[] = {L->tab.X, L->tab.S, L->tab.tag, L->mask_w, L->q_w, L->pre, L->arena};
  for (void *p : dev)
    if (p) (void)hipFree(p);
  for (int k = 0; k < LBA_KW; ++k) {
    if (L->kf_ids[k]) (void)hipFree(L->kf_ids[k]);
    if (L->kf_pl[k]) (void)hipFree(L->kf_pl[k]);
    if (L->kf_pr[k]) (void)hipFree(L->kf_pr[k]);
  }
  if (L->h_res) (void)hipHostFree(L->h_res);
  for (int32_t *p : L->pool)
    if (p) (void)hipFree(p);
  if (L->d_map) (void)hipFree(L->d_map);
  if (L->d_map_all) (void)hipFree(L->d_map_all);
  delete L;
  s->lba = nullptr;
}

static int lba_tab_alloc(vo_ctx *c, LmTab *t, int bits) {
  const size_t slots = (size_t)1 << bits;
  memset(t, 0, sizeof(*t));
  t->mask = (int)(slots - 1);
  VO_CHECK_HIP(c, vo_dev_malloc(c, (void **)&t->X, sizeof(float) * 3 * slots));
  VO_CHECK_HIP(c, vo_dev_malloc(c, (void **)&t->S, slots));
  VO_CHECK_HIP(c, vo_dev_malloc(c, (void **)&t->tag, sizeof(int32_t) * slots));
  VO_CHECK_HIP(c, hipMemsetAsync(t->tag, 0xFF, sizeof(int32_t) * slots, c->stream));
  VO_CHECK_HIP(c, hipMemsetAsync(t->S, 0, slots, c->stream));
  return VO_OK;
}
static void lba_tab_release(LmTab *t) {
  void *dev[] = {t->X, t->S, t->tag};
  for (void *p : dev)
    if (p) (void)hipFree(p);
  memset(t, 0, sizeof(*t));
}
static int lba_tab_reserve(vo_svo *s, long long id_hi) {
  vo_ctx *c = s->c;
  vo_svo_lba *L = s->lba;
  int bits = L->tab_bits;
  while (bits < LBA_TAB_BITS && id_hi - L->id_lo > ((long long)1 << bits)) ++bits;
  if (bits == L->tab_bits) return VO_OK;
  LmTab nt;
  const int rc = lba_tab_alloc(c, &nt, bits);
  if (rc < 0) {
    lba_tab_release(&nt);
    return rc;
  }
  hipLaunchKernelGGL(lba_tab_rehash_kernel, dim3((unsigned)((L->tab.mask + 256) / 256)), dim3(256), 0, c->stream, L->tab, nt);
  VO_CHECK_HIP(c, hipGetLastError());
  VO_CHECK_HIP(c, hipStreamSynchronize(c->stream));
  lba_tab_release(&L->tab);
  L->tab = nt;
  L->tab_bits = bits;
  return VO_OK;
}
static int lba_scratch_reserve(vo_svo *s, size_t ids) {
  vo_ctx *c = s->c;
  vo_svo_lba *L = s->lba;
  if (ids <= L->span_cap) return VO_OK;
  size_t want = L->span_cap ? L->span_cap : (size_t)LBA_SPAN_FIRST;
  while (want < ids) want *= 2;
  if (L->span_cap) VO_CHECK_HIP(c, hipStreamSynchronize(c->stream));
  void *old[] = {L->mask_w, L->q_w, L->pre};
  for (void *q : old)
    if (q) (void)hipFree(q);
  L->mask_w = L->q_w = nullptr;
  L->pre = nullptr;
  L->span_cap = 0;
  VO_CHECK_HIP(c, vo_dev_malloc(c, (void **)&L->mask_w, sizeof(int) * want));
  VO_CHECK_HIP(c, vo_dev_malloc(c, (void **)&L->q_w, sizeof(int) * want * (size_t)s->prm.kf_window));
  VO_CHECK_HIP(c, vo_dev_malloc(c, (void **)&L->pre, sizeof(unsigned long long) * (want + want / LBA_QWG + 1)));
  VO_CHECK_HIP(c, hipMemsetAsync(L->mask_w, 0, sizeof(int) * want, c->stream));
  L->span_cap = want;
  return VO_OK;
}
static int lba_pool_reserve(vo_svo *s, size_t n) {
  vo_svo_lba *L = s->lba;
  if (!L->pool.empty() && L->pool_used + n <= LBA_POOL_CHUNK) return VO_OK;
  int32_t *chunk = nullptr;
  VO_CHECK_HIP(s->c, vo_dev_malloc(s->c, (void **)&chunk, sizeof(int32_t) * LBA_POOL_CHUNK));
  L->pool.push_back(chunk);
  L->pool_fill.push_back(0);
  L->pool_used = 0;
  return VO_OK;
}

static void lba_make_layout(LbaLayout *l, int kf_window, int cap) {
  Arena ar;
  const int No = std::max(kf_window - 2, 1);
  const size_t E = (size_t)kf_window * cap, E_opt = (size_t)No * cap, M_ub = E, nobs_ub = 2 * E, ns_ub = E_opt, maxn = (size_t)cap;
  l->E_max = E;
  l->Eopt_max = E_opt;
  l->No_max = No;
  l->maxn = cap;
  l->n_err_max = (int)((M_ub + 64 / SBA_LQ - 1) / (64 / SBA_LQ));
  l->res_bytes = sizeof(double) * (16 * LBA_KW + 16) + sizeof(int) * (16 + 4);
  l->oT = ar.take(l->res_bytes);
  l->oAvg = l->oT + sizeof(double) * 16 * LBA_KW;
  l->oFl = l->oAvg + sizeof(double) * 16;
  l->oDyn = l->oFl + sizeof(int) * 16;
  l->oOpt = ar.take(sizeof(int) * LBA_KW);
  l->oOfr = ar.take(sizeof(int) * (No + 1));
  l->oX = ar.take(sizeof(double) * 3 * (M_ub + 1));
  l->oOp = ar.take(sizeof(int) * (M_ub + 1));
  l->oOf = ar.take(sizeof(int) * (nobs_ub + 2));
  l->oOr = ar.take(nobs_ub + 2);
  l->oPx = ar.take(sizeof(double) * 2 * (nobs_ub + 2));
  l->oSp = ar.take(sizeof(int) * (M_ub + 1));
  l->oSj = ar.take(sizeof(int) * (ns_ub + 1));
  l->oSb = ar.take(sizeof(int) * (ns_ub + 1));
  l->oSl = ar.take(sizeof(int) * (ns_ub + 1));
  l->oPop = ar.take(sizeof(int) * 2 * (No + 1));
  l->oPo = ar.take(sizeof(int) * 2 * maxn * No);
  l->oPl = ar.take(sizeof(int) * 2 * maxn * No);
  l->oPsp = ar.take(sizeof(int) * 2 * (No + 1));
  l->oPs = ar.take(sizeof(int) * maxn * No);
  l->oPp = ar.take(sizeof(int) * 2 * ((size_t)No * No + 1));
  l->oPa = ar.take(sizeof(int) * maxn * No * No);
  l->oPb = ar.take(sizeof(int) * maxn * No * No);
  l->oUid = ar.take(sizeof(int32_t) * (M_ub + 1));
  l->oLm = ar.take(sizeof(int) * (M_ub + 1));
  l->in_end = ar.off;
  SbaDev d;
  l->total = vo_sba_place_work(&d, nullptr, l->in_end, M_ub, ns_ub, No, 10, l->n_err_max);
}

static int lba_enqueue(vo_svo *s, const LbaWin &w, int maxn, size_t M_ub, const LbaHead &head, const LbaRef &ref, const SvoTrackSet &t,
                       int n, int max_iter, const double **res, uint32_t seq = 0, bool *delivered = nullptr) {
  vo_ctx *c = s->c;
  vo_svo_lba *L = s->lba;
  const LbaLayout &lay = L->lay;
  hipStream_t st = c->stream;
  const int nk = w.nk, No = w.No;
  const double inv_scale = ref.inv_scale;
  const int n_err = std::max(1, (int)((M_ub + 64 / SBA_LQ - 1) / (64 / SBA_LQ)));
  SbaDev d;
  memset(&d, 0, sizeof(d));
  uint8_t *base = L->arena;
  vo_sba_place_work(&d, base, lay.in_end, lay.E_max, lay.Eopt_max, lay.No_max, max_iter, lay.n_err_max);
  d.n_err = n_err;
  LbaProb p;
  memset(&p, 0, sizeof(p));
  p.T = (double *)(base + lay.oT);
  p.opt_index = (int *)(base + lay.oOpt);
  p.opt_frame = (int *)(base + lay.oOfr);
  p.X = (double *)(base + lay.oX);
  p.obs_ptr = (int *)(base + lay.oOp);
  p.obs_frame = (int *)(base + lay.oOf);
  p.obs_right = base + lay.oOr;
  p.px = (double *)(base + lay.oPx);
  p.slot_ptr = (int *)(base + lay.oSp);
  p.slot_j = (int *)(base + lay.oSj);
  p.slot_bobs = (int *)(base + lay.oSb);
  p.slot_lm = (int *)(base + lay.oSl);
  p.pose_obs_ptr = (int *)(base + lay.oPop);
  p.pose_obs_end = p.pose_obs_ptr + (lay.No_max + 1);
  p.pose_obs = (int *)(base + lay.oPo);
  p.pose_lm = (int *)(base + lay.oPl);
  p.pose_slot_ptr = (int *)(base + lay.oPsp);
  p.pose_slot_end = p.pose_slot_ptr + (lay.No_max + 1);
  p.pose_slot = (int *)(base + lay.oPs);
  p.pair_ptr = (int *)(base + lay.oPp);
  p.pair_end = p.pair_ptr + ((size_t)lay.No_max * lay.No_max + 1);
  p.pair_a = (int *)(base + lay.oPa);
  p.pair_b = (int *)(base + lay.oPb);
  p.flags = (int *)(base + lay.oFl);
  p.avg_err = (double *)(base + lay.oAvg);
  p.dyn = (int *)(base + lay.oDyn);
  p.used_id = (int32_t *)(base + lay.oUid);
  p.lm_mask = (int *)(base + lay.oLm);
  p.mask_w = L->mask_w;
  p.q_w = L->q_w;
  p.pre = L->pre;
  p.wg_tot = L->pre + L->span_cap;
  p.pose_obs_stride = 2 * lay.maxn;
  p.pose_slot_stride = lay.maxn;
  p.pair_stride = lay.maxn;
  p.max_iter = max_iter;
  hipLaunchKernelGGL(lba_scatter_kernel, dim3((maxn + 255) / 256, nk), dim3(256), 0, st, w, L->mask_w, L->q_w);
  const int n_wg = (w.W + LBA_QWG - 1) / LBA_QWG;
  hipLaunchKernelGGL(lba_qualify_kernel, dim3(n_wg), dim3(LBA_QWG), 0, st, w, L->tab, p);
  hipLaunchKernelGGL(lba_scan_kernel, dim3(1), dim3(1024), 0, st, w, p, head, n_wg);
  hipLaunchKernelGGL(lba_fill_kernel, dim3((w.W + 255) / 256), dim3(256), 0, st, w, L->tab, p, ref);
  hipLaunchKernelGGL(lba_lists_kernel, dim3(No + No * (No + 1) / 2), dim3(1024), 0, st, w, p);
  VO_CHECK_HIP(c, hipGetLastError());
  d.n_frames = nk;
  d.n_opt = No;
  d.stereo = s->mono ? 0 : 1;
  d.max_iter = max_iter;
  d.dyn = p.dyn;
  for (int k = 0; k < 4; ++k) {
    d.Kl[k] = (double)s->prm.frame.Kl[k];
    d.Kr[k] = (double)s->prm.frame.Kr[k];
  }
  {
    double T_lr[16];
    to_d(s->prm.frame.T_lr, T_lr);
    for (int r = 0; r < 3; ++r) T_lr[r * 4 + 3] *= inv_scale;
    for (int i = 0; i < 3; ++i)
      for (int j = 0; j < 3; ++j) d.R_rl[i * 3 + j] = T_lr[j * 4 + i];
    for (int i = 0; i < 3; ++i)
      d.t_rl[i] = (-d.R_rl[i * 3]) * T_lr[3] + ((-d.R_rl[i * 3 + 1]) * T_lr[7] + (-d.R_rl[i * 3 + 2]) * T_lr[11]);
  }
  d.thres_huber = 0.5;
  d.lambda = 0.00001;
  d.T = p.T;
  d.opt_index = p.opt_index;
  d.opt_frame = p.opt_frame;
  d.X = p.X;
  d.obs_ptr = p.obs_ptr;
  d.obs_frame = p.obs_frame;
  d.obs_right = p.obs_right;
  d.obs_px = p.px;
  d.slot_ptr = p.slot_ptr;
  d.slot_j = p.slot_j;
  d.slot_bobs = p.slot_bobs;
  d.slot_lm = p.slot_lm;
  d.pose_obs_ptr = p.pose_obs_ptr;
  d.pose_obs_end = p.pose_obs_end;
  d.pose_obs = p.pose_obs;
  d.pose_lm = p.pose_lm;
  d.pose_slot_ptr = p.pose_slot_ptr;
  d.pose_slot_end = p.pose_slot_end;
  d.pose_slot = p.pose_slot;
  d.pair_ptr = p.pair_ptr;
  d.pair_end = p.pair_end;
  d.pair_a = p.pair_a;
  d.pair_b = p.pair_b;
  d.avg_err = p.avg_err;
  d.flags = p.flags;
  if (seq) {
    d.res_host = (uint32_t *)L->h_res;
    d.res_src = (const uint32_t *)p.T;
    d.res_words = (int)(lay.res_bytes / 4);
    d.res_seq_word = LBA_SEQ_WORD;
    d.res_seq = seq;
    if (delivered) *delivered = vo_sba_delivers_result(c, d);
    if (!vo_sba_delivers_result(c, d)) d.res_host = nullptr;
  }
  vo_prof_begin(c, VO_K_AUX);
  {
    const int rc = vo_sba_enqueue_iterations(c, d, max_iter);
    if (rc < 0) return rc;
  }
  vo_prof_end(c);
  hipLaunchKernelGGL(lba_writeback_kernel, dim3((unsigned)((M_ub + 255) / 256)), dim3(256), 0, st, p, L->tab, ref);
  hipLaunchKernelGGL(lba_refresh_kernel, dim3((std::max(n, 1) + 255) / 256), dim3(256), 0, st, t, n, L->tab, s->mono);
  VO_CHECK_HIP(c, hipGetLastError());
  *res = p.T;
  return VO_OK;
}

static int lba_warm_up(vo_svo *s) {
  vo_ctx *c = s->c;
  vo_svo_lba *L = s->lba;
  VO_CHECK_HIP(c, hipMemsetAsync(L->arena, 0, L->lay.total, c->stream));
  LbaHead head;
  LbaRef ref;
  memset(&head, 0, sizeof(head));
  memset(&ref, 0, sizeof(ref));
  for (int k = 0; k < 4; ++k) ref.Tjw_ref[5 * k] = ref.Twj_ref[5 * k] = 1.0;
  ref.inv_scale = 0.1;
  ref.pose_scale = 10.0;
  for (int nk = 3; nk <= s->prm.kf_window; ++nk) {
    LbaWin w;
    memset(&w, 0, sizeof(w));
    w.nk = nk;
    w.No = nk - 2;
    w.kw = s->prm.kf_window;
    w.opk = s->mono ? 1 : 2;
    w.W = 1;
    for (int j = 0; j < nk; ++j) {
      w.ids[j] = L->kf_ids[0];
      w.pl[j] = L->kf_pl[0];
      w.pr[j] = L->kf_pr[0];
      w.opt[j] = j < 2 ? -1 : j - 2;
      if (j >= 2) {
        w.optf[j - 2] = j;
        w.optmask |= 1 << j;
      }
      for (int k = 0; k < 4; ++k) head.T_jw[16 * j + 5 * k] = 1.0;
    }
    const double *res = nullptr;
    const int rc = lba_enqueue(s, w, 1, 1, head, ref, s->ts[0], 0, 2, &res);
    if (rc < 0) return rc;
  }
  hipLaunchKernelGGL(lba_keyframe_kernel, dim3(1), dim3(256), 0, c->stream, s->ts[0], 0, L->tab, L->kf_ids[0], L->kf_pl[0], L->kf_pr[0],
                     L->pool.back());
  L->seq = 1;
  hipLaunchKernelGGL(lba_result_kernel, dim3(1), dim3(256), 0, c->stream, (const uint32_t *)L->arena, (uint32_t *)L->h_res, 16, L->seq);
  VO_CHECK_HIP(c, hipGetLastError());
  return VO_OK;
}

int vo_svo_lba_init(vo_svo *s) {
  vo_ctx *c = s->c;
  if (s->prm.kf_window > LBA_KW) VO_FAIL(c, VO_ERR_CAPACITY, "keyframe window of %d (at most %d)", s->prm.kf_window, LBA_KW);
  vo_svo_lba *L = new vo_svo_lba();
  s->lba = L;
  L->tab_bits = LBA_TAB_FIRST_BITS;
  int rc = lba_tab_alloc(c, &L->tab, L->tab_bits);
  if (rc < 0) return rc;
  for (int k = 0; k < s->prm.kf_window; ++k) {
    VO_CHECK_HIP(c, vo_dev_malloc(c, (void **)&L->kf_ids[k], sizeof(int32_t) * (size_t)s->cap));
    VO_CHECK_HIP(c, vo_dev_malloc(c, (void **)&L->kf_pl[k], sizeof(float) * 2 * (size_t)s->cap));
    VO_CHECK_HIP(c, vo_dev_malloc(c, (void **)&L->kf_pr[k], sizeof(float) * 2 * (size_t)s->cap));
  }
  VO_CHECK_HIP(c, vo_host_malloc(c, (void **)&L->h_res, 4096, hipHostMallocDefault));
  memset(L->h_res, 0, 4096);
  VO_CHECK_HIP(c, vo_dev_malloc(c, (void **)&L->d_map, sizeof(float) * 3 * (size_t)s->cap));
  rc = lba_pool_reserve(s, (size_t)s->cap);
  if (rc < 0) return rc;
  if (s->prm.local_ba && s->prm.kf_window >= 3) {
    lba_make_layout(&L->lay, s->prm.kf_window, s->cap);
    VO_CHECK_HIP(c, vo_dev_malloc(c, (void **)&L->arena, L->lay.total));
    size_t first = (size_t)LBA_SPAN_FIRST;
    while (first < 2 * (size_t)s->prm.kf_window * (size_t)s->cap) first *= 2;
    rc = lba_scratch_reserve(s, first);
    if (rc < 0) return rc;
    rc = lba_warm_up(s);
    if (rc < 0) return rc;
  }
  VO_CHECK_HIP(c, hipStreamSynchronize(c->stream));
  return VO_OK;
}

int vo_svo_lba_update_points(vo_svo *s, const SvoTrackSet &ts, int n) {
  vo_ctx *c = s->c;
  if (!s->lba || n <= 0) return VO_OK;
  hipLaunchKernelGGL(lba_table_update_kernel, dim3((n + 255) / 256), dim3(256), 0, c->stream, ts, n, s->lba->tab);
  VO_CHECK_HIP(c, hipGetLastError());
  return VO_OK;
}

size_t vo_svo_lba_bytes(const vo_svo *s) {
  const vo_svo_lba *L = s->lba;
  if (!L) return 0;
  size_t b = ((size_t)L->tab.mask + 1) * 17 + (size_t)s->prm.kf_window * (size_t)s->cap * 20 + sizeof(float) * 3 * (size_t)s->cap;
  b += L->pool.size() * LBA_POOL_CHUNK * sizeof(int32_t) + L->map_all_cap * 12;
  if (L->arena) b += L->lay.total;
  b += L->span_cap * (12 + 4 * (size_t)s->prm.kf_window) + (L->span_cap / LBA_QWG + 1) * 8;
  return b;
}

int vo_svo_local_ba(vo_svo *s, vo_svo_frame_info *info, int id_min) {
  vo_ctx *c = s->c;
  const int n = s->n;
  SvoTrackSet &t = s->ts[s->cur];
  static const bool trace = getenv("VO_SVO_TRACE") != nullptr;
  const double t_0 = trace ? lba_now() : 0.0;
  hipStream_t st = c->stream;
  vo_svo_lba *L = s->lba;
  if (!L) VO_FAIL(c, VO_ERR_INVALID, "StereoVO: the keyframe storage was not initialised");
  std::vector<SvoKeyframe> &win = s->keyframes;
  const int nk = (int)win.size();
  SvoKeyframe &kf = win.back();
  {
    unsigned used = 0;
    for (int j = 0; j + 1 < nk; ++j) used |= 1u << win[j].ring;
    int r = 0;
    while (used & (1u << r)) ++r;
    kf.ring = r;
    kf.n = n;
    kf.id_min = id_min;
    kf.global = (int)s->kf_all.size();
  }
  if (n > 0) {
    if (!L->id_seen || (long long)id_min < L->id_lo) L->id_lo = id_min;
    L->id_seen = true;
    const int rc = lba_tab_reserve(s, (long long)c->next_landmark_id);
    if (rc < 0) return rc;
  }
  {
    const int rc = lba_pool_reserve(s, (size_t)n);
    if (rc < 0) return rc;
    vo_svo::SvoKfAll rec;
    memcpy(rec.T_wc, kf.T_wc, sizeof(rec.T_wc));
    rec.n = n;
    rec.d_ids = L->pool.back() + L->pool_used;
    L->pool_used += (size_t)n;
    L->pool_fill.back() = L->pool_used;
    s->kf_all.push_back(rec);
  }
  if (n > 0) {
    hipLaunchKernelGGL(lba_keyframe_kernel, dim3((n + 255) / 256), dim3(256), 0, st, t, n, L->tab, L->kf_ids[kf.ring], L->kf_pl[kf.ring],
                       L->kf_pr[kf.ring], const_cast<int32_t *>(s->kf_all.back().d_ids));
    VO_CHECK_HIP(c, hipGetLastError());
  }
  if (!s->prm.local_ba) return VO_OK;
  if (nk < 3) return VO_OK;
  const double POSE_SCALE = 10.0, inv_scale = 1.0 / POSE_SCALE;
  const LbaLayout &lay = L->lay;
  LbaWin w;
  memset(&w, 0, sizeof(w));
  w.nk = nk;
  w.No = nk - 2;
  w.kw = s->prm.kf_window;
  w.opk = s->mono ? 1 : 2;
  w.base = win.front().id_min;
  const long long span = (long long)c->next_landmark_id - (long long)w.base;
  if (span > LBA_SPAN_MAX) VO_FAIL(c, VO_ERR_CAPACITY, "local BA: the window spans %lld landmark ids (at most %d)", span, LBA_SPAN_MAX);
  w.W = (int)span;
  {
    const int rc = lba_scratch_reserve(s, (size_t)std::max(w.W, 0));
    if (rc < 0) return rc;
  }
  size_t E = 0, E_opt = 0;
  int maxn = 1;
  for (int j = 0; j < nk; ++j) {
    w.n[j] = win[j].n;
    w.ids[j] = L->kf_ids[win[j].ring];
    w.pl[j] = L->kf_pl[win[j].ring];
    w.pr[j] = L->kf_pr[win[j].ring];
    w.opt[j] = j < 2 ? -1 : j - 2;
    if (j >= 2) {
      w.optf[j - 2] = j;
      w.optmask |= 1 << j;
      E_opt += (size_t)win[j].n;
    }
    E += (size_t)win[j].n;
    maxn = std::max(maxn, win[j].n);
  }
  if (w.W <= 0 || E == 0) return VO_OK;
  if (E >= ((size_t)1 << LBA_PK_KF))
    VO_FAIL(c, VO_ERR_CAPACITY, "local BA: %zu keyframe entries exceed the packed counters", E);
  if (E > lay.E_max || E_opt > lay.Eopt_max || maxn > lay.maxn || nk - 2 > lay.No_max)
    VO_FAIL(c, VO_ERR_CAPACITY, "local BA: the window (%zu entries) exceeds the arena laid out at construction", E);
  const int max_iter = 10;
  const size_t M_ub = std::min((size_t)w.W, E);
  LbaRef ref;
  LbaHead head;
  memset(&head, 0, sizeof(head));
  to_d(win.front().T_wc, ref.Twj_ref);
  inv_se3d(ref.Twj_ref, ref.Tjw_ref);
  ref.inv_scale = inv_scale;
  ref.pose_scale = POSE_SCALE;
  for (int j = 0; j < nk; ++j) {
    float Tjw_f[16];
    double Tjw[16];
    svo_inv_se3(win[j].T_wc, Tjw_f);
    to_d(Tjw_f, Tjw);
    mul44d(Tjw, ref.Twj_ref, &head.T_jw[16 * j]);
    for (int r = 0; r < 3; ++r) head.T_jw[16 * j + r * 4 + 3] *= inv_scale;
  }
  const double *res_dev = nullptr;
  bool delivered = false;
  L->seq = L->seq + 1 == 0 ? 1 : L->seq + 1;
  {
    const int rc = lba_enqueue(s, w, maxn, M_ub, head, ref, t, n, max_iter, &res_dev, L->seq, &delivered);
    if (rc < 0) return rc;
  }
  double *o_T = (double *)L->h_res, *o_e = o_T + 16 * LBA_KW;
  int *o_f = (int *)(o_e + 16), *o_d = o_f + 16;
  if (!delivered)
    hipLaunchKernelGGL(lba_result_kernel, dim3(1), dim3(256), 0, st, (const uint32_t *)res_dev, (uint32_t *)L->h_res, (int)(lay.res_bytes / 4),
                       L->seq);
  VO_CHECK_HIP(c, hipGetLastError());
  const double t_1 = trace ? lba_now() : 0.0;
  {
    volatile const uint32_t *seqp = (volatile const uint32_t *)L->h_res + LBA_SEQ_WORD;
    bool seen = false;
    timespec p0;
    clock_gettime(CLOCK_MONOTONIC, &p0);
    for (int spin = 0; !seen; ++spin) {
      if (*seqp == L->seq) {
        seen = true;
        break;
      }
      if ((spin & 255) == 255) {
        timespec p1;
        clock_gettime(CLOCK_MONOTONIC, &p1);
        if ((p1.tv_sec - p0.tv_sec) * 1e9 + (p1.tv_nsec - p0.tv_nsec) > 2e7) break;
      }
      if (c->dbg[VO_OPT_POLL_YIELD]) sched_yield();
#if defined(__x86_64__)
      else __builtin_ia32_pause();
#endif
    }
    __atomic_thread_fence(__ATOMIC_ACQUIRE);
    if (!seen) VO_CHECK_HIP(c, hipStreamSynchronize(st));
  }
  const double t_2 = trace ? lba_now() : 0.0;
  if (o_d[0] <= 0) return VO_OK;
  if (o_f[0] & 1) VO_FAIL(c, VO_ERR_LBA_NAN, "In LBA, pose becomes nan!");
  if (o_f[0] & 2) VO_FAIL(c, VO_ERR_LBA_NAN, "Local BA NAN!");
  if (info) {
    info->lba_ran = 1;
    info->lba_err_first = o_e[0];
    info->lba_err_last = o_e[max_iter - 1];
    info->lba_landmarks = o_d[0];
    info->lba_observations = o_d[1];
  }
  for (int j = 0; j < nk; ++j) {
    if (w.opt[j] < 0) continue;
    double T[16], Tjw[16], Twj_orig[16], dT[16];
    for (int k = 0; k < 16; ++k) T[k] = o_T[16 * j + k];
    for (int r = 0; r < 3; ++r) T[r * 4 + 3] *= POSE_SCALE;
    mul44d(T, ref.Tjw_ref, Tjw);
    to_d(win[j].T_wc, Twj_orig);
    mul44d(Twj_orig, Tjw, dT);
    const double tn = sqrt(dT[3] * dT[3] + (dT[7] * dT[7] + dT[11] * dT[11]));
    if (tn > 50) VO_FAIL(c, VO_ERR_LBA_NAN, "local BA: large update!");
    float Tf[16];
    for (int k = 0; k < 12; ++k) Tf[k] = (float)Tjw[k];
    Tf[12] = Tf[13] = Tf[14] = 0.0f;
    Tf[15] = 1.0f;
    svo_inv_se3(Tf, win[j].T_wc);
    memcpy(s->kf_all[win[j].global].T_wc, win[j].T_wc, sizeof(win[j].T_wc));
  }
  if (trace) {
    const double t_3 = lba_now();
    L->tt[0] += t_1 - t_0;
    L->tt[1] += t_2 - t_1;
    L->tt[2] += t_3 - t_2;
    if ((++L->n_calls % 10) == 0)
      fprintf(stderr, "[lba] per call (us): host build + enqueue %.0f  device (build + solve) %.0f  write-back %.0f  (M=%d obs=%d slots=%d, span %d)\n",
              L->tt[0] / L->n_calls, L->tt[1] / L->n_calls, L->tt[2] / L->n_calls, o_d[0], o_d[1], o_d[2], w.W);
  }
  return VO_OK;
}

extern "C" int vo_svo_device_bytes(const vo_svo *s, size_t *bytes) {
  if (!s || !bytes) return VO_ERR_INVALID;
  *bytes = vo_svo_lba_bytes(s);
  return VO_OK;
}

extern "C" int vo_svo_keyframe_count(vo_svo *s, int *n_keyframes) {
  if (!s || !n_keyframes) return VO_ERR_INVALID;
  *n_keyframes = (int)s->kf_all.size();
  return VO_OK;
}

extern "C" int vo_svo_get_keyframe(vo_svo *s, int j, float T_wc[16], float *mappoints, int cap, int *n_points) {
  if (!s || j < 0 || j >= (int)s->kf_all.size()) return VO_ERR_INVALID;
  vo_ctx *c = s->c;
  if (s->pending) VO_FAIL(c, VO_ERR_INVALID, "call vo_svo_result first");
  const vo_svo::SvoKfAll &k = s->kf_all[j];
  if (T_wc) memcpy(T_wc, k.T_wc, sizeof(k.T_wc));
  if (n_points) *n_points = k.n;
  if (!mappoints || k.n == 0) return VO_OK;
  if (k.n > cap) VO_FAIL(c, VO_ERR_CAPACITY, "keyframe %d has %d related landmarks, room for %d", j, k.n, cap);
  VO_CHECK_HIP(c, hipSetDevice(c->device));
  vo_svo_lba *L = s->lba;
  hipLaunchKernelGGL(lba_mappoints_kernel, dim3((k.n + 255) / 256), dim3(256), 0, c->stream, k.d_ids, k.n, L->tab, L->d_map);
  VO_CHECK_HIP(c, hipGetLastError());
  VO_CHECK_HIP(c, hipMemcpyAsync(mappoints, L->d_map, sizeof(float) * 3 * (size_t)k.n, hipMemcpyDeviceToHost, c->stream));
  VO_CHECK_HIP(c, hipStreamSynchronize(c->stream));
  return VO_OK;
}

extern "C" int vo_svo_get_keyframes(vo_svo *s, float *T_wc, int32_t *n_points, float *mappoints, size_t cap_points,
                                    size_t *total_points) {
  if (!s) return VO_ERR_INVALID;
  vo_ctx *c = s->c;
  if (s->pending) VO_FAIL(c, VO_ERR_INVALID, "call vo_svo_result first");
  size_t total = 0;
  for (size_t j = 0; j < s->kf_all.size(); ++j) {
    if (T_wc) memcpy(T_wc + 16 * j, s->kf_all[j].T_wc, sizeof(float) * 16);
    if (n_points) n_points[j] = s->kf_all[j].n;
    total += (size_t)s->kf_all[j].n;
  }
  if (total_points) *total_points = total;
  if (!mappoints || total == 0) return VO_OK;
  if (total > cap_points) VO_FAIL(c, VO_ERR_CAPACITY, "%zu map points, room for %zu", total, cap_points);
  VO_CHECK_HIP(c, hipSetDevice(c->device));
  vo_svo_lba *L = s->lba;
  if (L->map_all_cap < total) {
    VO_CHECK_HIP(c, hipStreamSynchronize(c->stream));
    if (L->d_map_all) (void)hipFree(L->d_map_all);
    L->d_map_all = nullptr;
    L->map_all_cap = 0;
    const size_t want = total + (total >> 1) + 4096;
    VO_CHECK_HIP(c, vo_dev_malloc(c, (void **)&L->d_map_all, sizeof(float) * 3 * want));
    L->map_all_cap = want;
  }
  size_t off = 0;
  for (size_t q = 0; q < L->pool.size(); ++q) {
    const size_t m = L->pool_fill[q];
    if (!m) continue;
    hipLaunchKernelGGL(lba_mappoints_kernel, dim3((unsigned)((m + 255) / 256)), dim3(256), 0, c->stream, L->pool[q], (int)m, L->tab,
                       L->d_map_all + 3 * off);
    off += m;
  }
  VO_CHECK_HIP(c, hipGetLastError());
  VO_CHECK_HIP(c, hipMemcpyAsync(mappoints, L->d_map_all, sizeof(float) * 3 * total, hipMemcpyDeviceToHost, c->stream));
  VO_CHECK_HIP(c, hipStreamSynchronize(c->stream));
  return VO_OK;
}
```

Baseline: 2708.

## Fuse local BA problem build into mark, qualify, and single build kernel

Merges the local BA setup into three kernels instead of six. The keyframe write folds into the scatter (mark) kernel, qualify stores a qualified mask, and one build kernel does the head rows, fill and pose/pair list construction, with per-wave prefix offsets replacing the separate scan kernel. This is meant to cut kernel launches and serial dependencies on the per-keyframe BA path. The old sequence stays behind a debug switch; the trade-off is redundant per-wave offset sums and more complex indexing.

```diff
diff --git a/include/vo_hip.h b/include/vo_hip.h
--- a/include/vo_hip.h
+++ b/include/vo_hip.h
@@ -193,7 +193,7 @@
 
 enum { VO_DBG_FAIL_JOIN = 0, VO_DBG_CONC_GRID = 1, VO_DBG_SBA_LDS_SOLVE = 2, VO_DBG_SKIP_DETECT = 3, VO_OPT_POLL_YIELD = 4,
        VO_DBG_MVO_HOST_ADVANCE = 5, VO_DBG_STAGED_DETECT = 6, VO_DBG_CANDS_IN_FRAME = 7, VO_DBG_SBA_SPLIT = 8,
-       VO_DBG_SDP_STAGE = 9, VO_DBG_SDW_FORM = 10, VO_DBG_COUNT = 11 };
+       VO_DBG_SDP_STAGE = 9, VO_DBG_SDW_FORM = 10, VO_DBG_LBA_BUILD_SPLIT = 11, VO_DBG_COUNT = 12 };
 int vo_debug_set(vo_ctx *ctx, int key, int value);
 int vo_debug_allocation_count(const vo_ctx *ctx, long long *count);
 
diff --git a/visual_odometry_ros_amd/api.py b/visual_odometry_ros_amd/api.py
--- a/visual_odometry_ros_amd/api.py
+++ b/visual_odometry_ros_amd/api.py
@@ -499,7 +499,7 @@
         if os.environ.get("VO_TEST_SWITCHES") == "1":
             for key, name in ((0, "VO_DEBUG_FAIL_JOIN"), (1, "VO_CONC_GRID"), (2, "VO_SBA_LDS_SOLVE"), (3, "VO_DEBUG_SKIP_DETECT"),
                               (5, "VO_MVO_HOST_ADVANCE"), (6, "VO_STAGED_DETECT"), (7, "VO_CANDS_IN_FRAME"),
-                              (8, "VO_SBA_SPLIT")):
+                              (8, "VO_SBA_SPLIT"), (11, "VO_LBA_BUILD_SPLIT")):
                 v = os.environ.get(name)
                 if v:
                     self.debug_set(key, int(v) if v.lstrip("-").isdigit() else 1)
@@ -508,6 +508,7 @@
     DBG_FAIL_JOIN, DBG_CONC_GRID, DBG_SBA_LDS_SOLVE, DBG_SKIP_DETECT, OPT_POLL_YIELD, DBG_MVO_HOST_ADVANCE, DBG_STAGED_DETECT, DBG_CANDS_IN_FRAME = 0, 1, 2, 3, 4, 5, 6, 7
     DBG_SBA_SPLIT = 8
     DBG_SDP_STAGE = 9
+    DBG_LBA_BUILD_SPLIT = 11
 
     @property
     def sum_order(self):
diff --git a/visual_odometry_ros_amd/csrc/lba_build_device.hpp b/visual_odometry_ros_amd/csrc/lba_build_device.hpp
--- /dev/null
+++ b/visual_odometry_ros_amd/csrc/lba_build_device.hpp
@@ -0,0 +1,447 @@
+#pragma once
+#include <stddef.h>
+#include <stdint.h>
+
+#define LBA_KW 16
+
+struct LbaTrackView {
+  const float *pts_l, *pts_r, *Xw;
+  const uint8_t *flags;
+  const int32_t *ids;
+};
+struct LmTab {
+  float *X;
+  uint8_t *S;
+  int32_t *tag;
+  int mask;
+};
+struct LbaWin {
+  int nk, No, W, base;
+  int kw;
+  int opk;
+  int n[LBA_KW];
+  const int32_t *ids[LBA_KW];
+  const float *pl[LBA_KW], *pr[LBA_KW];
+  int opt[LBA_KW];
+  int optf[LBA_KW];
+  int optmask;
+};
+struct LbaProb {
+  double *T, *X, *px;
+  int *opt_index, *opt_frame, *obs_ptr, *obs_frame, *slot_ptr, *slot_j, *slot_bobs, *slot_lm;
+  uint8_t *obs_right;
+  int *pose_obs_ptr, *pose_obs_end, *pose_obs, *pose_lm, *pose_slot_ptr, *pose_slot_end, *pose_slot;
+  int *pair_ptr, *pair_end, *pair_a, *pair_b;
+  int *flags, *dyn;
+  double *avg_err;
+  int32_t *used_id;
+  int *lm_mask;
+  int *mask_w, *q_w;
+  int *qmask;
+  unsigned long long *pre, *wg_tot;
+  int pose_obs_stride, pose_slot_stride, pair_stride, max_iter;
+};
+struct LbaKfDst {
+  int32_t *ids;
+  float *pl, *pr;
+  int32_t *all_ids;
+};
+
+__device__ __forceinline__ int32_t lba_keyframe_entry(const LbaTrackView &ts, int k, const LmTab &tab, const LbaKfDst &d) {
+  const int32_t id = ts.ids[k];
+  const int t = id & tab.mask;
+  const uint8_t dead = tab.tag[t] == id ? (uint8_t)(tab.S[t] & 2) : (uint8_t)0;
+  tab.X[3 * (size_t)t] = ts.Xw[3 * k];
+  tab.X[3 * (size_t)t + 1] = ts.Xw[3 * k + 1];
+  tab.X[3 * (size_t)t + 2] = ts.Xw[3 * k + 2];
+  tab.S[t] = (uint8_t)(dead | ((ts.flags[k] & VO_LM_TRIANGULATED) ? 1 : 0) | ((ts.flags[k] & VO_LM_BUNDLED) ? 4 : 0));
+  tab.tag[t] = id;
+  d.ids[k] = id;
+  d.all_ids[k] = id;
+  d.pl[2 * k] = ts.pts_l[2 * k];
+  d.pl[2 * k + 1] = ts.pts_l[2 * k + 1];
+  d.pr[2 * k] = ts.pts_r[2 * k];
+  d.pr[2 * k + 1] = ts.pts_r[2 * k + 1];
+  return id;
+}
+__global__ void lba_keyframe_kernel(LbaTrackView ts, int n, LmTab tab, LbaKfDst d) {
+  const int k = blockIdx.x * blockDim.x + threadIdx.x;
+  if (k >= n) return;
+  (void)lba_keyframe_entry(ts, k, tab, d);
+}
+
+__global__ void lba_scatter_kernel(LbaWin w, int *mask_w, int *q_w) {
+  const int j = blockIdx.y, q = blockIdx.x * blockDim.x + threadIdx.x;
+  if (q >= w.n[j]) return;
+  const int idx = w.ids[j][q] - w.base;
+  if ((unsigned)idx >= (unsigned)w.W) return;
+  atomicOr(&mask_w[idx], 1 << j);
+  q_w[(size_t)idx * w.kw + j] = q;
+}
+
+__global__ void lba_mark_kernel(LbaTrackView ts, LbaWin w, LmTab tab, LbaKfDst d, int *mask_w, int *q_w) {
+  const int j = blockIdx.y, q = blockIdx.x * blockDim.x + threadIdx.x;
+  if (q >= w.n[j]) return;
+  const int32_t id = j == w.nk - 1 ? lba_keyframe_entry(ts, q, tab, d) : w.ids[j][q];
+  const int idx = id - w.base;
+  if ((unsigned)idx >= (unsigned)w.W) return;
+  atomicOr(&mask_w[idx], 1 << j);
+  q_w[(size_t)idx * w.kw + j] = q;
+}
+
+__device__ __forceinline__ int lba_block_scan(int v, int *s_w, int &total) {
+  const int tid = threadIdx.x, lane = tid & 63, wave = tid >> 6;
+  int inc = v;
+#pragma unroll
+  for (int off = 1; off < 64; off <<= 1) {
+    const int t = __shfl_up(inc, off);
+    if (lane >= off) inc += t;
+  }
+  __syncthreads();
+  if (lane == 63) s_w[wave] = inc;
+  __syncthreads();
+  int before = 0, tot = 0;
+#pragma unroll
+  for (int k = 0; k < 16; ++k) {
+    const int c = s_w[k];
+    before += k < wave ? c : 0;
+    tot += c;
+  }
+  total = tot;
+  return before + inc - v;
+}
+
+template <int NW>
+__device__ __forceinline__ unsigned long long lba_block_scan64(unsigned long long v, unsigned long long *s_w,
+                                                               unsigned long long &total) {
+  const int tid = threadIdx.x, lane = tid & 63, wave = tid >> 6;
+  unsigned long long inc = v;
+#pragma unroll
+  for (int off = 1; off < 64; off <<= 1) {
+    const unsigned long long t = __shfl_up(inc, off);
+    if (lane >= off) inc += t;
+  }
+  __syncthreads();
+  if (lane == 63) s_w[wave] = inc;
+  __syncthreads();
+  unsigned long long before = 0, tot = 0;
+#pragma unroll
+  for (int k = 0; k < NW; ++k) {
+    const unsigned long long c = s_w[k];
+    before += k < wave ? c : 0;
+    tot += c;
+  }
+  total = tot;
+  return before + inc - v;
+}
+#define LBA_PK_KF 20
+#define LBA_PK_SL 42
+#define LBA_QWG 256
+__device__ __forceinline__ void lba_unpack(unsigned long long pk, int &i, int &kf0, int &s0) {
+  i = (int)(pk & ((1ull << LBA_PK_KF) - 1));
+  kf0 = (int)((pk >> LBA_PK_KF) & ((1ull << (LBA_PK_SL - LBA_PK_KF)) - 1));
+  s0 = (int)(pk >> LBA_PK_SL);
+}
+
+template <bool QM>
+__global__ __launch_bounds__(LBA_QWG) void lba_qualify_kernel(LbaWin w, LmTab tab, LbaProb p) {
+  __shared__ unsigned long long s_w[LBA_QWG / 64];
+  const int idx = blockIdx.x * LBA_QWG + threadIdx.x;
+  int m = idx < w.W ? p.mask_w[idx] : 0;
+  if (m) {
+    if (QM) p.mask_w[idx] = 0;
+    const int32_t id = w.base + idx;
+    const int t = id & tab.mask;
+    const uint8_t st = tab.tag[t] == id ? tab.S[t] : (uint8_t)0;
+    if (!((st & 1) && !(st & 2)) || w.opk * __popc(m) < 2) {
+      m = 0;
+      if (!QM) p.mask_w[idx] = 0;
+    }
+  }
+  if (QM && idx < w.W) p.qmask[idx] = m;
+  const unsigned long long v =
+      m ? 1ull | ((unsigned long long)__popc(m) << LBA_PK_KF) | ((unsigned long long)__popc(m & w.optmask) << LBA_PK_SL) : 0ull;
+  unsigned long long total;
+  const unsigned long long ex = lba_block_scan64<LBA_QWG / 64>(v, s_w, total);
+  if (idx < w.W) p.pre[idx] = ex;
+  if (threadIdx.x == 0) p.wg_tot[blockIdx.x] = total;
+}
+
+struct LbaHead {
+  double T_jw[16 * LBA_KW];
+};
+__device__ __forceinline__ void lba_head_rows(const LbaWin &w, const LbaProb &p, const LbaHead &h) {
+  const int tid = threadIdx.x, nt = blockDim.x;
+  for (int k = tid; k < 16 * w.nk; k += nt) p.T[k] = h.T_jw[k];
+  for (int k = tid; k < w.nk; k += nt) p.opt_index[k] = w.opt[k];
+  for (int k = tid; k < w.No; k += nt) p.opt_frame[k] = w.optf[k];
+  for (int k = tid; k < 16; k += nt) p.flags[k] = 0;
+  for (int k = tid; k <= p.max_iter; k += nt) p.avg_err[k] = 0.0;
+}
+__device__ __forceinline__ void lba_head_counts(const LbaWin &w, const LbaProb &p, unsigned long long total) {
+  int t_lm, t_kf, t_sl;
+  lba_unpack(total, t_lm, t_kf, t_sl);
+  p.dyn[0] = t_lm;
+  p.dyn[1] = w.opk * t_kf;
+  p.dyn[2] = t_sl;
+  p.obs_ptr[t_lm] = w.opk * t_kf;
+  p.slot_ptr[t_lm] = t_sl;
+}
+__global__ __launch_bounds__(1024) void lba_scan_kernel(LbaWin w, LbaProb p, LbaHead h, int n_wg) {
+  __shared__ unsigned long long s_w[16];
+  const int tid = threadIdx.x;
+  lba_head_rows(w, p, h);
+  const int chunk = (n_wg + 1023) / 1024, i0 = tid * chunk, i1 = min(i0 + chunk, n_wg);
+  unsigned long long c = 0;
+  for (int g = i0; g < i1; ++g) c += p.wg_tot[g];
+  unsigned long long total, off = lba_block_scan64<16>(c, s_w, total);
+  for (int g = i0; g < i1; ++g) {
+    const unsigned long long t = p.wg_tot[g];
+    p.wg_tot[g] = off;
+    off += t;
+  }
+  if (tid == 0) lba_head_counts(w, p, total);
+}
+
+struct LbaRef {
+  double Tjw_ref[16], Twj_ref[16], inv_scale, pose_scale;
+};
+__device__ __forceinline__ void lba_fill_row(const LbaWin &w, const LmTab &tab, const LbaProb &p, const LbaRef &r, int idx, int m,
+                                             unsigned long long pk) {
+  int i, kf0, s0;
+  lba_unpack(pk, i, kf0, s0);
+  const int32_t id = w.base + idx;
+  const int t = id & tab.mask;
+  p.used_id[i] = id;
+  p.lm_mask[i] = m;
+  const double Xd[3] = {(double)tab.X[3 * (size_t)t], (double)tab.X[3 * (size_t)t + 1], (double)tab.X[3 * (size_t)t + 2]};
+#pragma unroll
+  for (int k = 0; k < 3; ++k) {
+    const double xr = (r.Tjw_ref[k * 4 + 0] * Xd[0] + (r.Tjw_ref[k * 4 + 1] * Xd[1] + r.Tjw_ref[k * 4 + 2] * Xd[2])) + r.Tjw_ref[k * 4 + 3];
+    p.X[3 * (size_t)i + k] = xr * r.inv_scale;
+  }
+  p.obs_ptr[i] = w.opk * kf0;
+  p.slot_ptr[i] = s0;
+  int rr = 0, rs = 0;
+  for (int mm = m; mm; mm &= mm - 1) {
+    const int j = __ffs(mm) - 1;
+    const int q = p.q_w[(size_t)idx * w.kw + j];
+    const int o = w.opk * (kf0 + rr);
+    p.obs_frame[o] = j;
+    p.obs_right[o] = 0;
+    p.px[2 * (size_t)o] = (double)w.pl[j][2 * q];
+    p.px[2 * (size_t)o + 1] = (double)w.pl[j][2 * q + 1];
+    if (w.opk == 2) {
+      p.obs_frame[o + 1] = j;
+      p.obs_right[o + 1] = 1;
+      p.px[2 * (size_t)o + 2] = (double)w.pr[j][2 * q];
+      p.px[2 * (size_t)o + 3] = (double)w.pr[j][2 * q + 1];
+    }
+    if (w.opt[j] >= 0) {
+      const int s = s0 + rs;
+      p.slot_j[s] = w.opt[j];
+      p.slot_bobs[s] = o + w.opk - 1;
+      p.slot_lm[s] = i;
+      ++rs;
+    }
+    ++rr;
+  }
+}
+__global__ void lba_fill_kernel(LbaWin w, LmTab tab, LbaProb p, LbaRef r) {
+  const int idx = blockIdx.x * blockDim.x + threadIdx.x;
+  if (idx >= w.W) return;
+  const int m = p.mask_w[idx];
+  if (!m) return;
+  p.mask_w[idx] = 0;
+  lba_fill_row(w, tab, p, r, idx, m, p.pre[idx] + p.wg_tot[idx / LBA_QWG]);
+}
+
+__global__ __launch_bounds__(1024) void lba_lists_kernel(LbaWin w, LbaProb p) {
+  __shared__ int s_w[16];
+  const int tid = threadIdx.x, M = p.dyn[0], No = w.No;
+  const int chunk = (M + 1023) / 1024, i0 = tid * chunk, i1 = min(i0 + chunk, M);
+  int u = blockIdx.x;
+  if (u < No) {
+    const int f = w.optf[u], bit = 1 << f;
+    int cnt = 0;
+    for (int i = i0; i < i1; ++i) cnt += (p.lm_mask[i] & bit) ? 1 : 0;
+    int total, off = lba_block_scan(cnt, s_w, total);
+    const int Bo = u * p.pose_obs_stride, Bs = u * p.pose_slot_stride;
+    for (int i = i0; i < i1; ++i) {
+      const int m = p.lm_mask[i];
+      if (!(m & bit)) continue;
+      const int o = p.obs_ptr[i] + w.opk * __popc(m & (bit - 1));
+      for (int e = 0; e < w.opk; ++e) {
+        p.pose_obs[Bo + w.opk * off + e] = o + e;
+        p.pose_lm[Bo + w.opk * off + e] = i;
+      }
+      p.pose_slot[Bs + off] = p.slot_ptr[i] + __popc(m & w.optmask & (bit - 1));
+      ++off;
+    }
+    if (tid == 0) {
+      p.pose_obs_ptr[u] = Bo;
+      p.pose_obs_end[u] = Bo + w.opk * total;
+      p.pose_slot_ptr[u] = Bs;
+      p.pose_slot_end[u] = Bs + total;
+    }
+    return;
+  }
+  u -= No;
+  int a = 0;
+  while (u >= No - a) {
+    u -= No - a;
+    ++a;
+  }
+  const int b = a + u, jk = a * No + b;
+  const int ba = 1 << w.optf[a], bb = 1 << w.optf[b], both = ba | bb;
+  int cnt = 0;
+  for (int i = i0; i < i1; ++i) cnt += ((p.lm_mask[i] & both) == both) ? 1 : 0;
+  int total, off = lba_block_scan(cnt, s_w, total);
+  const int Bp = jk * p.pair_stride;
+  for (int i = i0; i < i1; ++i) {
+    const int m = p.lm_mask[i];
+    if ((m & both) != both) continue;
+    const int sp = p.slot_ptr[i];
+    p.pair_a[Bp + off] = sp + __popc(m & w.optmask & (ba - 1));
+    p.pair_b[Bp + off] = sp + __popc(m & w.optmask & (bb - 1));
+    ++off;
+  }
+  if (tid == 0) {
+    p.pair_ptr[jk] = Bp;
+    p.pair_end[jk] = Bp + total;
+  }
+}
+
+__device__ __forceinline__ unsigned long long lba_wave_offset(const unsigned long long *wg_tot, int g_end) {
+  unsigned long long c = 0;
+  for (int g = threadIdx.x & 63; g < g_end; g += 64) c += wg_tot[g];
+#pragma unroll
+  for (int off = 32; off; off >>= 1) c += __shfl_xor(c, off);
+  return c;
+}
+
+#ifndef LBA_BWG
+#define LBA_BWG 1024
+#endif
+#ifndef LBA_LB
+#define LBA_LB 8
+#endif
+static_assert((64 * LBA_LB) % LBA_QWG == 0 && LBA_QWG % 64 == 0, "a batch is whole qualify groups, a step lies inside one");
+__global__ __launch_bounds__(LBA_BWG) void lba_build_kernel(LbaWin w, LmTab tab, LbaProb p, LbaHead h, LbaRef r, int n_wg) {
+  __shared__ int s_cnt[LBA_BWG / 64];
+  const int tid = threadIdx.x, lane = tid & 63, wave = tid >> 6, No = w.No;
+  const int n_lists = No + No * (No + 1) / 2;
+  if ((int)blockIdx.x >= n_lists) {
+    const int fb = (int)blockIdx.x - n_lists;
+    if (fb == 0) {
+      lba_head_rows(w, p, h);
+      if (wave == 0) {
+        const unsigned long long total = lba_wave_offset(p.wg_tot, n_wg);
+        if (lane == 0) lba_head_counts(w, p, total);
+      }
+    }
+    const int idx = fb * LBA_BWG + tid;
+    const int m = idx < w.W ? p.qmask[idx] : 0;
+    if (!__ballot(m != 0)) return;
+    const unsigned long long off = lba_wave_offset(p.wg_tot, (idx - lane) / LBA_QWG);
+    if (m) lba_fill_row(w, tab, p, r, idx, m, p.pre[idx] + off);
+    return;
+  }
+  int u = blockIdx.x, need, ba = 0, bb = 0, jk = 0;
+  const bool pose_list = u < No;
+  if (pose_list) {
+    need = 1 << w.optf[u];
+  } else {
+    u -= No;
+    int a = 0;
+    while (u >= No - a) {
+      u -= No - a;
+      ++a;
+    }
+    const int b = a + u;
+    jk = a * No + b;
+    ba = 1 << w.optf[a];
+    bb = 1 << w.optf[b];
+    need = ba | bb;
+  }
+  const int nw = (int)blockDim.x >> 6, batch = 64 * LBA_LB;
+  const int per = (((w.W + nw - 1) / nw) + batch - 1) / batch * batch;
+  const int a0 = min(wave * per, w.W), a1 = min(a0 + per, w.W);
+  int cnt = 0;
+  for (int c0 = a0; c0 < a1; c0 += batch) {
+    int m[LBA_LB];
+#pragma unroll
+    for (int k = 0; k < LBA_LB; ++k) {
+      const int idx = c0 + 64 * k + lane;
+      m[k] = idx < a1 ? p.qmask[idx] : 0;
+    }
+#pragma unroll
+    for (int k = 0; k < LBA_LB; ++k) cnt += (m[k] & need) == need ? 1 : 0;
+  }
+#pragma unroll
+  for (int off = 32; off; off >>= 1) cnt += __shfl_xor(cnt, off);
+  if (lane == 0) s_cnt[wave] = cnt;
+  __syncthreads();
+  int pos = 0, total = 0;
+  for (int k = 0; k < nw; ++k) {
+    const int c = s_cnt[k];
+    pos += k < wave ? c : 0;
+    total += c;
+  }
+  if (tid == 0) {
+    if (pose_list) {
+      const int Bo = u * p.pose_obs_stride, Bs = u * p.pose_slot_stride;
+      p.pose_obs_ptr[u] = Bo;
+      p.pose_obs_end[u] = Bo + w.opk * total;
+      p.pose_slot_ptr[u] = Bs;
+      p.pose_slot_end[u] = Bs + total;
+    } else {
+      p.pair_ptr[jk] = jk * p.pair_stride;
+      p.pair_end[jk] = jk * p.pair_stride + total;
+    }
+  }
+  if (cnt == 0) return;
+  unsigned long long goff = lba_wave_offset(p.wg_tot, a0 / LBA_QWG);
+  const int Bo = u * p.pose_obs_stride, Bs = u * p.pose_slot_stride, Bp = jk * p.pair_stride;
+  for (int c0 = a0; c0 < a1; c0 += batch) {
+    const int g0 = c0 / LBA_QWG;
+    unsigned long long gq[LBA_LB * 64 / LBA_QWG + 1];
+    gq[0] = goff;
+#pragma unroll
+    for (int q = 0; q < LBA_LB * 64 / LBA_QWG; ++q) gq[q + 1] = gq[q] + (g0 + q < n_wg ? p.wg_tot[g0 + q] : 0ull);
+    goff = gq[LBA_LB * 64 / LBA_QWG];
+    int m[LBA_LB];
+    unsigned long long vote[LBA_LB], pk[LBA_LB];
+#pragma unroll
+    for (int k = 0; k < LBA_LB; ++k) {
+      const int idx = c0 + 64 * k + lane;
+      m[k] = idx < a1 ? p.qmask[idx] : 0;
+    }
+#pragma unroll
+    for (int k = 0; k < LBA_LB; ++k) {
+      const bool hit = (m[k] & need) == need;
+      vote[k] = __ballot(hit);
+      pk[k] = hit ? p.pre[c0 + 64 * k + lane] : 0ull;
+    }
+#pragma unroll
+    for (int k = 0; k < LBA_LB; ++k) {
+      if ((m[k] & need) == need) {
+        int i, kf0, s0;
+        lba_unpack(pk[k] + gq[64 * k / LBA_QWG], i, kf0, s0);
+        const int at = pos + __popcll(vote[k] & ((1ull << lane) - 1));
+        if (pose_list) {
+          const int o = w.opk * kf0 + w.opk * __popc(m[k] & (need - 1));
+          for (int e = 0; e < w.opk; ++e) {
+            p.pose_obs[Bo + w.opk * at + e] = o + e;
+            p.pose_lm[Bo + w.opk * at + e] = i;
+          }
+          p.pose_slot[Bs + at] = s0 + __popc(m[k] & w.optmask & (need - 1));
+        } else {
+          p.pair_a[Bp + at] = s0 + __popc(m[k] & w.optmask & (ba - 1));
+          p.pair_b[Bp + at] = s0 + __popc(m[k] & w.optmask & (bb - 1));
+        }
+      }
+      pos += __popcll(vote[k]);
+    }
+  }
+}
diff --git a/visual_odometry_ros_amd/csrc/stereo_vo_lba.hip b/visual_odometry_ros_amd/csrc/stereo_vo_lba.hip
--- a/visual_odometry_ros_amd/csrc/stereo_vo_lba.hip
+++ b/visual_odometry_ros_amd/csrc/stereo_vo_lba.hip
@@ -8,6 +8,7 @@
 
 #include "sba_device.hpp"
 #include "stereo_vo.hpp"
+#include "lba_build_device.hpp"
 
 static double lba_now() {
   timespec ts;
@@ -43,62 +44,13 @@
   D[15] = 1.0;
 }
 
-#define LBA_KW 16
 #define LBA_TAB_FIRST_BITS 18
 #define LBA_TAB_BITS 24
 #define LBA_SPAN_MAX (1 << LBA_TAB_BITS)
 #define LBA_SPAN_FIRST (1 << 16)
 
-struct LmTab {
-  float *X;
-  uint8_t *S;
-  int32_t *tag;
-  int mask;
-};
-struct LbaWin {
-  int nk, No, W, base;
-  int kw;
-  int opk;
-  int n[LBA_KW];
-  const int32_t *ids[LBA_KW];
-  const float *pl[LBA_KW], *pr[LBA_KW];
-  int opt[LBA_KW];
-  int optf[LBA_KW];
-  int optmask;
-};
-struct LbaProb {
-  double *T, *X, *px;
-  int *opt_index, *opt_frame, *obs_ptr, *obs_frame, *slot_ptr, *slot_j, *slot_bobs, *slot_lm;
-  uint8_t *obs_right;
-  int *pose_obs_ptr, *pose_obs_end, *pose_obs, *pose_lm, *pose_slot_ptr, *pose_slot_end, *pose_slot;
-  int *pair_ptr, *pair_end, *pair_a, *pair_b;
-  int *flags, *dyn;
-  double *avg_err;
-  int32_t *used_id;
-  int *lm_mask;
-  int *mask_w, *q_w;
-  unsigned long long *pre, *wg_tot;
-  int pose_obs_stride, pose_slot_stride, pair_stride, max_iter;
-};
-
-__global__ void lba_keyframe_kernel(SvoTrackSet ts, int n, LmTab tab, int32_t *kf_ids, float *kf_pl, float *kf_pr, int32_t *all_ids) {
-  const int k = blockIdx.x * blockDim.x + threadIdx.x;
-  if (k >= n) return;
-  const int32_t id = ts.ids[k];
-  const int t = id & tab.mask;
-  const uint8_t dead = tab.tag[t] == id ? (uint8_t)(tab.S[t] & 2) : (uint8_t)0;
-  tab.X[3 * (size_t)t] = ts.Xw[3 * k];
-  tab.X[3 * (size_t)t + 1] = ts.Xw[3 * k + 1];
-  tab.X[3 * (size_t)t + 2] = ts.Xw[3 * k + 2];
-  tab.S[t] = (uint8_t)(dead | ((ts.flags[k] & VO_LM_TRIANGULATED) ? 1 : 0) | ((ts.flags[k] & VO_LM_BUNDLED) ? 4 : 0));
-  tab.tag[t] = id;
-  kf_ids[k] = id;
-  all_ids[k] = id;
-  kf_pl[2 * k] = ts.pts_l[2 * k];
-  kf_pl[2 * k + 1] = ts.pts_l[2 * k + 1];
-  kf_pr[2 * k] = ts.pts_r[2 * k];
-  kf_pr[2 * k + 1] = ts.pts_r[2 * k + 1];
-}
+static_assert(sizeof(LbaWin) + sizeof(LmTab) + sizeof(LbaProb) + sizeof(LbaHead) + sizeof(LbaRef) + 64 <= 4096,
+              "lba_build_kernel takes all of them by value: a kernel's arguments are 4 KB at most");
 
 __global__ void lba_table_update_kernel(SvoTrackSet ts, int n, LmTab tab) {
   const int k = blockIdx.x * blockDim.x + threadIdx.x;
@@ -110,222 +62,6 @@
   tab.X[3 * (size_t)t + 1] = ts.Xw[3 * k + 1];
   tab.X[3 * (size_t)t + 2] = ts.Xw[3 * k + 2];
   tab.S[t] = (uint8_t)((tab.S[t] & 2) | ((ts.flags[k] & VO_LM_TRIANGULATED) ? 1 : 0) | ((ts.flags[k] & VO_LM_BUNDLED) ? 4 : 0));
-}
-
-__global__ void lba_scatter_kernel(LbaWin w, int *mask_w, int *q_w) {
-  const int j = blockIdx.y, q = blockIdx.x * blockDim.x + threadIdx.x;
-  if (q >= w.n[j]) return;
-  const int idx = w.ids[j][q] - w.base;
-  if ((unsigned)idx >= (unsigned)w.W) return;
-  atomicOr(&mask_w[idx], 1 << j);
-  q_w[(size_t)idx * w.kw + j] = q;
-}
-
-__device__ __forceinline__ int lba_block_scan(int v, int *s_w, int &total) {
-  const int tid = threadIdx.x, lane = tid & 63, wave = tid >> 6;
-  int inc = v;
-#pragma unroll
-  for (int off = 1; off < 64; off <<= 1) {
-    const int t = __shfl_up(inc, off);
-    if (lane >= off) inc += t;
-  }
-  __syncthreads();
-  if (lane == 63) s_w[wave] = inc;
-  __syncthreads();
-  int before = 0, tot = 0;
-#pragma unroll
-  for (int k = 0; k < 16; ++k) {
-    const int c = s_w[k];
-    before += k < wave ? c : 0;
-    tot += c;
-  }
-  total = tot;
-  return before + inc - v;
-}
-
-template <int NW>
-__device__ __forceinline__ unsigned long long lba_block_scan64(unsigned long long v, unsigned long long *s_w,
-                                                               unsigned long long &total) {
-  const int tid = threadIdx.x, lane = tid & 63, wave = tid >> 6;
-  unsigned long long inc = v;
-#pragma unroll
-  for (int off = 1; off < 64; off <<= 1) {
-    const unsigned long long t = __shfl_up(inc, off);
-    if (lane >= off) inc += t;
-  }
-  __syncthreads();
-  if (lane == 63) s_w[wave] = inc;
-  __syncthreads();
-  unsigned long long before = 0, tot = 0;
-#pragma unroll
-  for (int k = 0; k < NW; ++k) {
-    const unsigned long long c = s_w[k];
-    before += k < wave ? c : 0;
-    tot += c;
-  }
-  total = tot;
-  return before + inc - v;
-}
-#define LBA_PK_KF 20
-#define LBA_PK_SL 42
-#define LBA_QWG 256
-
-__global__ __launch_bounds__(LBA_QWG) void lba_qualify_kernel(LbaWin w, LmTab tab, LbaProb p) {
-  __shared__ unsigned long long s_w[LBA_QWG / 64];
-  const int idx = blockIdx.x * LBA_QWG + threadIdx.x;
-  int m = idx < w.W ? p.mask_w[idx] : 0;
-  if (m) {
-    const int32_t id = w.base + idx;
-    const int t = id & tab.mask;
-    const uint8_t st = tab.tag[t] == id ? tab.S[t] : (uint8_t)0;
-    if (!((st & 1) && !(st & 2)) || w.opk * __popc(m) < 2) {
-      m = 0;
-      p.mask_w[idx] = 0;
-    }
-  }
-  const unsigned long long v =
-      m ? 1ull | ((unsigned long long)__popc(m) << LBA_PK_KF) | ((unsigned long long)__popc(m & w.optmask) << LBA_PK_SL) : 0ull;
-  unsigned long long total;
-  const unsigned long long ex = lba_block_scan64<LBA_QWG / 64>(v, s_w, total);
-  if (idx < w.W) p.pre[idx] = ex;
-  if (threadIdx.x == 0) p.wg_tot[blockIdx.x] = total;
-}
-
-struct LbaHead {
-  double T_jw[16 * LBA_KW];
-};
-__global__ __launch_bounds__(1024) void lba_scan_kernel(LbaWin w, LbaProb p, LbaHead h, int n_wg) {
-  __shared__ unsigned long long s_w[16];
-  const int tid = threadIdx.x;
-  for (int k = tid; k < 16 * w.nk; k += 1024) p.T[k] = h.T_jw[k];
-  if (tid < w.nk) p.opt_index[tid] = w.opt[tid];
-  if (tid < w.No) p.opt_frame[tid] = w.optf[tid];
-  if (tid < 16) p.flags[tid] = 0;
-  if (tid <= p.max_iter) p.avg_err[tid] = 0.0;
-  const int chunk = (n_wg + 1023) / 1024, i0 = tid * chunk, i1 = min(i0 + chunk, n_wg);
-  unsigned long long c = 0;
-  for (int g = i0; g < i1; ++g) c += p.wg_tot[g];
-  unsigned long long total, off = lba_block_scan64<16>(c, s_w, total);
-  for (int g = i0; g < i1; ++g) {
-    const unsigned long long t = p.wg_tot[g];
-    p.wg_tot[g] = off;
-    off += t;
-  }
-  if (tid == 0) {
-    const int t_lm = (int)(total & ((1ull << LBA_PK_KF) - 1)), t_kf = (int)((total >> LBA_PK_KF) & ((1ull << (LBA_PK_SL - LBA_PK_KF)) - 1));
-    const int t_sl = (int)(total >> LBA_PK_SL);
-    p.dyn[0] = t_lm;
-    p.dyn[1] = w.opk * t_kf;
-    p.dyn[2] = t_sl;
-    p.obs_ptr[t_lm] = w.opk * t_kf;
-    p.slot_ptr[t_lm] = t_sl;
-  }
-}
-
-struct LbaRef {
-  double Tjw_ref[16], Twj_ref[16], inv_scale, pose_scale;
-};
-__global__ void lba_fill_kernel(LbaWin w, LmTab tab, LbaProb p, LbaRef r) {
-  const int idx = blockIdx.x * blockDim.x + threadIdx.x;
-  if (idx >= w.W) return;
-  const int m = p.mask_w[idx];
-  if (!m) return;
-  p.mask_w[idx] = 0;
-  const unsigned long long pk = p.pre[idx] + p.wg_tot[idx / LBA_QWG];
-  const int i = (int)(pk & ((1ull << LBA_PK_KF) - 1)), kf0 = (int)((pk >> LBA_PK_KF) & ((1ull << (LBA_PK_SL - LBA_PK_KF)) - 1));
-  const int s0 = (int)(pk >> LBA_PK_SL);
-  const int32_t id = w.base + idx;
-  const int t = id & tab.mask;
-  p.used_id[i] = id;
-  p.lm_mask[i] = m;
-  const double Xd[3] = {(double)tab.X[3 * (size_t)t], (double)tab.X[3 * (size_t)t + 1], (double)tab.X[3 * (size_t)t + 2]};
-#pragma unroll
-  for (int k = 0; k < 3; ++k) {
-    const double xr = (r.Tjw_ref[k * 4 + 0] * Xd[0] + (r.Tjw_ref[k * 4 + 1] * Xd[1] + r.Tjw_ref[k * 4 + 2] * Xd[2])) + r.Tjw_ref[k * 4 + 3];
-    p.X[3 * (size_t)i + k] = xr * r.inv_scale;
-  }
-  p.obs_ptr[i] = w.opk * kf0;
-  p.slot_ptr[i] = s0;
-  int rr = 0, rs = 0;
-  for (int mm = m; mm; mm &= mm - 1) {
-    const int j = __ffs(mm) - 1;
-    const int q = p.q_w[(size_t)idx * w.kw + j];
-    const int o = w.opk * (kf0 + rr);
-    p.obs_frame[o] = j;
-    p.obs_right[o] = 0;
-    p.px[2 * (size_t)o] = (double)w.pl[j][2 * q];
-    p.px[2 * (size_t)o + 1] = (double)w.pl[j][2 * q + 1];
-    if (w.opk == 2) {
-      p.obs_frame[o + 1] = j;
-      p.obs_right[o + 1] = 1;
-      p.px[2 * (size_t)o + 2] = (double)w.pr[j][2 * q];
-      p.px[2 * (size_t)o + 3] = (double)w.pr[j][2 * q + 1];
-    }
-    if (w.opt[j] >= 0) {
-      const int s = s0 + rs;
-      p.slot_j[s] = w.opt[j];
-      p.slot_bobs[s] = o + w.opk - 1;
-      p.slot_lm[s] = i;
-      ++rs;
-    }
-    ++rr;
-  }
-}
-
-__global__ __launch_bounds__(1024) void lba_lists_kernel(LbaWin w, LbaProb p) {
-  __shared__ int s_w[16];
-  const int tid = threadIdx.x, M = p.dyn[0], No = w.No;
-  const int chunk = (M + 1023) / 1024, i0 = tid * chunk, i1 = min(i0 + chunk, M);
-  int u = blockIdx.x;
-  if (u < No) {
-    const int f = w.optf[u], bit = 1 << f;
-    int cnt = 0;
-    for (int i = i0; i < i1; ++i) cnt += (p.lm_mask[i] & bit) ? 1 : 0;
-    int total, off = lba_block_scan(cnt, s_w, total);
-    const int Bo = u * p.pose_obs_stride, Bs = u * p.pose_slot_stride;
-    for (int i = i0; i < i1; ++i) {
-      const int m = p.lm_mask[i];
-      if (!(m & bit)) continue;
-      const int o = p.obs_ptr[i] + w.opk * __popc(m & (bit - 1));
-      for (int e = 0; e < w.opk; ++e) {
-        p.pose_obs[Bo + w.opk * off + e] = o + e;
-        p.pose_lm[Bo + w.opk * off + e] = i;
-      }
-      p.pose_slot[Bs + off] = p.slot_ptr[i] + __popc(m & w.optmask & (bit - 1));
-      ++off;
-    }
-    if (tid == 0) {
-      p.pose_obs_ptr[u] = Bo;
-      p.pose_obs_end[u] = Bo + w.opk * total;
-      p.pose_slot_ptr[u] = Bs;
-      p.pose_slot_end[u] = Bs + total;
-    }
-    return;
-  }
-  u -= No;
-  int a = 0;
-  while (u >= No - a) {
-    u -= No - a;
-    ++a;
-  }
-  const int b = a + u, jk = a * No + b;
-  const int ba = 1 << w.optf[a], bb = 1 << w.optf[b], both = ba | bb;
-  int cnt = 0;
-  for (int i = i0; i < i1; ++i) cnt += ((p.lm_mask[i] & both) == both) ? 1 : 0;
-  int total, off = lba_block_scan(cnt, s_w, total);
-  const int Bp = jk * p.pair_stride;
-  for (int i = i0; i < i1; ++i) {
-    const int m = p.lm_mask[i];
-    if ((m & both) != both) continue;
-    const int sp = p.slot_ptr[i];
-    p.pair_a[Bp + off] = sp + __popc(m & w.optmask & (ba - 1));
-    p.pair_b[Bp + off] = sp + __popc(m & w.optmask & (bb - 1));
-    ++off;
-  }
-  if (tid == 0) {
-    p.pair_ptr[jk] = Bp;
-    p.pair_end[jk] = Bp + total;
-  }
 }
 
 __global__ void lba_writeback_kernel(LbaProb p, LmTab tab, LbaRef r) {
@@ -421,6 +157,7 @@
   int32_t *kf_ids[LBA_KW] = {};
   float *kf_pl[LBA_KW] = {}, *kf_pr[LBA_KW] = {};
   int *mask_w = nullptr, *q_w = nullptr;
+  int *qmask = nullptr;
   unsigned long long *pre = nullptr;
   size_t span_cap = 0;
   uint8_t *arena = nullptr;
@@ -440,7 +177,7 @@
 void vo_svo_lba_free(vo_svo *s) {
   vo_svo_lba *L = s->lba;
   if (!L) return;
-  void *dev[] = {L->tab.X, L->tab.S, L->tab.tag, L->mask_w, L->q_w, L->pre, L->arena};
+  void *dev[] = {L->tab.X, L->tab.S, L->tab.tag, L->mask_w, L->q_w, L->qmask, L->pre, L->arena};
   for (void *p : dev)
     if (p) (void)hipFree(p);
   for (int k = 0; k < LBA_KW; ++k) {
@@ -501,14 +238,15 @@
   size_t want = L->span_cap ? L->span_cap : (size_t)LBA_SPAN_FIRST;
   while (want < ids) want *= 2;
   if (L->span_cap) VO_CHECK_HIP(c, hipStreamSynchronize(c->stream));
-  void *old[] = {L->mask_w, L->q_w, L->pre};
+  void *old[] = {L->mask_w, L->q_w, L->qmask, L->pre};
   for (void *q : old)
     if (q) (void)hipFree(q);
-  L->mask_w = L->q_w = nullptr;
+  L->mask_w = L->q_w = L->qmask = nullptr;
   L->pre = nullptr;
   L->span_cap = 0;
   VO_CHECK_HIP(c, vo_dev_malloc(c, (void **)&L->mask_w, sizeof(int) * want));
   VO_CHECK_HIP(c, vo_dev_malloc(c, (void **)&L->q_w, sizeof(int) * want * (size_t)s->prm.kf_window));
+  VO_CHECK_HIP(c, vo_dev_malloc(c, (void **)&L->qmask, sizeof(int) * want));
   VO_CHECK_HIP(c, vo_dev_malloc(c, (void **)&L->pre, sizeof(unsigned long long) * (want + want / LBA_QWG + 1)));
   VO_CHECK_HIP(c, hipMemsetAsync(L->mask_w, 0, sizeof(int) * want, c->stream));
   L->span_cap = want;
@@ -565,8 +303,9 @@
   l->total = vo_sba_place_work(&d, nullptr, l->in_end, M_ub, ns_ub, No, 10, l->n_err_max);
 }
 
-static int lba_enqueue(vo_svo *s, const LbaWin &w, int maxn, size_t M_ub, const LbaHead &head, const LbaRef &ref, const SvoTrackSet &t,
-                       int n, int max_iter, const double **res, uint32_t seq = 0, bool *delivered = nullptr) {
+static int lba_enqueue(vo_svo *s, bool split, const LbaKfDst &kfd, const LbaWin &w, int maxn, size_t M_ub, const LbaHead &head,
+                       const LbaRef &ref, const SvoTrackSet &t, int n, int max_iter, const double **res, uint32_t seq = 0,
+                       bool *delivered = nullptr) {
   vo_ctx *c = s->c;
   vo_svo_lba *L = s->lba;
   const LbaLayout &lay = L->lay;
@@ -617,12 +356,20 @@
   p.pose_slot_stride = lay.maxn;
   p.pair_stride = lay.maxn;
   p.max_iter = max_iter;
-  hipLaunchKernelGGL(lba_scatter_kernel, dim3((maxn + 255) / 256, nk), dim3(256), 0, st, w, L->mask_w, L->q_w);
-  const int n_wg = (w.W + LBA_QWG - 1) / LBA_QWG;
-  hipLaunchKernelGGL(lba_qualify_kernel, dim3(n_wg), dim3(LBA_QWG), 0, st, w, L->tab, p);
-  hipLaunchKernelGGL(lba_scan_kernel, dim3(1), dim3(1024), 0, st, w, p, head, n_wg);
-  hipLaunchKernelGGL(lba_fill_kernel, dim3((w.W + 255) / 256), dim3(256), 0, st, w, L->tab, p, ref);
-  hipLaunchKernelGGL(lba_lists_kernel, dim3(No + No * (No + 1) / 2), dim3(1024), 0, st, w, p);
+  p.qmask = L->qmask;
+  const int n_wg = (w.W + LBA_QWG - 1) / LBA_QWG, n_lists = No + No * (No + 1) / 2;
+  if (!split) {
+    const LbaTrackView tv = {t.pts_l, t.pts_r, t.Xw, t.flags, t.ids};
+    hipLaunchKernelGGL(lba_mark_kernel, dim3((maxn + 255) / 256, nk), dim3(256), 0, st, tv, w, L->tab, kfd, L->mask_w, L->q_w);
+    hipLaunchKernelGGL((lba_qualify_kernel<true>), dim3(n_wg), dim3(LBA_QWG), 0, st, w, L->tab, p);
+    hipLaunchKernelGGL(lba_build_kernel, dim3(n_lists + (w.W + LBA_BWG - 1) / LBA_BWG), dim3(LBA_BWG), 0, st, w, L->tab, p, head, ref, n_wg);
+  } else {
+    hipLaunchKernelGGL(lba_scatter_kernel, dim3((maxn + 255) / 256, nk), dim3(256), 0, st, w, L->mask_w, L->q_w);
+    hipLaunchKernelGGL((lba_qualify_kernel<false>), dim3(n_wg), dim3(LBA_QWG), 0, st, w, L->tab, p);
+    hipLaunchKernelGGL(lba_scan_kernel, dim3(1), dim3(1024), 0, st, w, p, head, n_wg);
+    hipLaunchKernelGGL(lba_fill_kernel, dim3((w.W + 255) / 256), dim3(256), 0, st, w, L->tab, p, ref);
+    hipLaunchKernelGGL(lba_lists_kernel, dim3(n_lists), dim3(1024), 0, st, w, p);
+  }
   VO_CHECK_HIP(c, hipGetLastError());
   d.n_frames = nk;
   d.n_opt = No;
@@ -702,6 +449,9 @@
   for (int k = 0; k < 4; ++k) ref.Tjw_ref[5 * k] = ref.Twj_ref[5 * k] = 1.0;
   ref.inv_scale = 0.1;
   ref.pose_scale = 10.0;
+  const LbaKfDst kfd = {L->kf_ids[0], L->kf_pl[0], L->kf_pr[0], L->pool.back()};
+  const SvoTrackSet &t0 = s->ts[0];
+  const LbaTrackView tv = {t0.pts_l, t0.pts_r, t0.Xw, t0.flags, t0.ids};
   for (int nk = 3; nk <= s->prm.kf_window; ++nk) {
     LbaWin w;
     memset(&w, 0, sizeof(w));
@@ -722,11 +472,10 @@
       for (int k = 0; k < 4; ++k) head.T_jw[16 * j + 5 * k] = 1.0;
     }
     const double *res = nullptr;
-    const int rc = lba_enqueue(s, w, 1, 1, head, ref, s->ts[0], 0, 2, &res);
+    const int rc = lba_enqueue(s, c->dbg[VO_DBG_LBA_BUILD_SPLIT] != 0, kfd, w, 1, 1, head, ref, s->ts[0], 0, 2, &res);
     if (rc < 0) return rc;
   }
-  hipLaunchKernelGGL(lba_keyframe_kernel, dim3(1), dim3(256), 0, c->stream, s->ts[0], 0, L->tab, L->kf_ids[0], L->kf_pl[0], L->kf_pr[0],
-                     L->pool.back());
+  hipLaunchKernelGGL(lba_keyframe_kernel, dim3(1), dim3(256), 0, c->stream, tv, 0, L->tab, kfd);
   L->seq = 1;
   hipLaunchKernelGGL(lba_result_kernel, dim3(1), dim3(256), 0, c->stream, (const uint32_t *)L->arena, (uint32_t *)L->h_res, 16, L->seq);
   VO_CHECK_HIP(c, hipGetLastError());
@@ -779,59 +528,25 @@
   size_t b = ((size_t)L->tab.mask + 1) * 17 + (size_t)s->prm.kf_window * (size_t)s->cap * 20 + sizeof(float) * 3 * (size_t)s->cap;
   b += L->pool.size() * LBA_POOL_CHUNK * sizeof(int32_t) + L->map_all_cap * 12;
   if (L->arena) b += L->lay.total;
-  b += L->span_cap * (12 + 4 * (size_t)s->prm.kf_window) + (L->span_cap / LBA_QWG + 1) * 8;
+  b += L->span_cap * (16 + 4 * (size_t)s->prm.kf_window) + (L->span_cap / LBA_QWG + 1) * 8;
   return b;
 }
 
-int vo_svo_local_ba(vo_svo *s, vo_svo_frame_info *info, int id_min) {
-  vo_ctx *c = s->c;
-  const int n = s->n;
-  SvoTrackSet &t = s->ts[s->cur];
-  static const bool trace = getenv("VO_SVO_TRACE") != nullptr;
-  const double t_0 = trace ? lba_now() : 0.0;
-  hipStream_t st = c->stream;
-  vo_svo_lba *L = s->lba;
-  if (!L) VO_FAIL(c, VO_ERR_INVALID, "StereoVO: the keyframe storage was not initialised");
-  std::vector<SvoKeyframe> &win = s->keyframes;
+static int lba_keyframe_alone(vo_svo *s, const SvoTrackSet &t, int n, const LbaKfDst &kfd) {
+  if (n <= 0) return VO_OK;
+  const LbaTrackView tv = {t.pts_l, t.pts_r, t.Xw, t.flags, t.ids};
+  hipLaunchKernelGGL(lba_keyframe_kernel, dim3((n + 255) / 256), dim3(256), 0, s->c->stream, tv, n, s->lba->tab, kfd);
+  VO_CHECK_HIP(s->c, hipGetLastError());
+  return VO_OK;
+}
+
+static int lba_window(vo_svo *s, LbaWin *wp, size_t *E_out, int *maxn_out) {
+  vo_ctx *c = s->c;
+  vo_svo_lba *L = s->lba;
+  const LbaLayout &lay = L->lay;
+  const std::vector<SvoKeyframe> &win = s->keyframes;
   const int nk = (int)win.size();
-  SvoKeyframe &kf = win.back();
-  {
-    unsigned used = 0;
-    for (int j = 0; j + 1 < nk; ++j) used |= 1u << win[j].ring;
-    int r = 0;
-    while (used & (1u << r)) ++r;
-    kf.ring = r;
-    kf.n = n;
-    kf.id_min = id_min;
-    kf.global = (int)s->kf_all.size();
-  }
-  if (n > 0) {
-    if (!L->id_seen || (long long)id_min < L->id_lo) L->id_lo = id_min;
-    L->id_seen = true;
-    const int rc = lba_tab_reserve(s, (long long)c->next_landmark_id);
-    if (rc < 0) return rc;
-  }
-  {
-    const int rc = lba_pool_reserve(s, (size_t)n);
-    if (rc < 0) return rc;
-    vo_svo::SvoKfAll rec;
-    memcpy(rec.T_wc, kf.T_wc, sizeof(rec.T_wc));
-    rec.n = n;
-    rec.d_ids = L->pool.back() + L->pool_used;
-    L->pool_used += (size_t)n;
-    L->pool_fill.back() = L->pool_used;
-    s->kf_all.push_back(rec);
-  }
-  if (n > 0) {
-    hipLaunchKernelGGL(lba_keyframe_kernel, dim3((n + 255) / 256), dim3(256), 0, st, t, n, L->tab, L->kf_ids[kf.ring], L->kf_pl[kf.ring],
-                       L->kf_pr[kf.ring], const_cast<int32_t *>(s->kf_all.back().d_ids));
-    VO_CHECK_HIP(c, hipGetLastError());
-  }
-  if (!s->prm.local_ba) return VO_OK;
-  if (nk < 3) return VO_OK;
-  const double POSE_SCALE = 10.0, inv_scale = 1.0 / POSE_SCALE;
-  const LbaLayout &lay = L->lay;
-  LbaWin w;
+  LbaWin &w = *wp;
   memset(&w, 0, sizeof(w));
   w.nk = nk;
   w.No = nk - 2;
@@ -861,11 +576,75 @@
     E += (size_t)win[j].n;
     maxn = std::max(maxn, win[j].n);
   }
+  *E_out = E;
+  *maxn_out = maxn;
   if (w.W <= 0 || E == 0) return VO_OK;
   if (E >= ((size_t)1 << LBA_PK_KF))
     VO_FAIL(c, VO_ERR_CAPACITY, "local BA: %zu keyframe entries exceed the packed counters", E);
   if (E > lay.E_max || E_opt > lay.Eopt_max || maxn > lay.maxn || nk - 2 > lay.No_max)
     VO_FAIL(c, VO_ERR_CAPACITY, "local BA: the window (%zu entries) exceeds the arena laid out at construction", E);
+  return VO_OK;
+}
+
+int vo_svo_local_ba(vo_svo *s, vo_svo_frame_info *info, int id_min) {
+  vo_ctx *c = s->c;
+  const int n = s->n;
+  SvoTrackSet &t = s->ts[s->cur];
+  static const bool trace = getenv("VO_SVO_TRACE") != nullptr;
+  const double t_0 = trace ? lba_now() : 0.0;
+  hipStream_t st = c->stream;
+  vo_svo_lba *L = s->lba;
+  if (!L) VO_FAIL(c, VO_ERR_INVALID, "StereoVO: the keyframe storage was not initialised");
+  std::vector<SvoKeyframe> &win = s->keyframes;
+  const int nk = (int)win.size();
+  SvoKeyframe &kf = win.back();
+  {
+    unsigned used = 0;
+    for (int j = 0; j + 1 < nk; ++j) used |= 1u << win[j].ring;
+    int r = 0;
+    while (used & (1u << r)) ++r;
+    kf.ring = r;
+    kf.n = n;
+    kf.id_min = id_min;
+    kf.global = (int)s->kf_all.size();
+  }
+  if (n > 0) {
+    if (!L->id_seen || (long long)id_min < L->id_lo) L->id_lo = id_min;
+    L->id_seen = true;
+    const int rc = lba_tab_reserve(s, (long long)c->next_landmark_id);
+    if (rc < 0) return rc;
+  }
+  {
+    const int rc = lba_pool_reserve(s, (size_t)n);
+    if (rc < 0) return rc;
+    vo_svo::SvoKfAll rec;
+    memcpy(rec.T_wc, kf.T_wc, sizeof(rec.T_wc));
+    rec.n = n;
+    rec.d_ids = L->pool.back() + L->pool_used;
+    L->pool_used += (size_t)n;
+    L->pool_fill.back() = L->pool_used;
+    s->kf_all.push_back(rec);
+  }
+  const LbaKfDst kfd = {L->kf_ids[kf.ring], L->kf_pl[kf.ring], L->kf_pr[kf.ring], const_cast<int32_t *>(s->kf_all.back().d_ids)};
+  if (!s->prm.local_ba || nk < 3) return lba_keyframe_alone(s, t, n, kfd);
+  const double POSE_SCALE = 10.0, inv_scale = 1.0 / POSE_SCALE;
+  LbaWin w;
+  size_t E = 0;
+  int maxn = 1;
+  {
+    const int rc = lba_window(s, &w, &E, &maxn);
+    if (rc < 0) {
+      (void)lba_keyframe_alone(s, t, n, kfd);
+      return rc;
+    }
+  }
+  if (w.W <= 0 || E == 0) return lba_keyframe_alone(s, t, n, kfd);
+  const bool split = c->dbg[VO_DBG_LBA_BUILD_SPLIT] != 0;
+  if (split) {
+    const int rc = lba_keyframe_alone(s, t, n, kfd);
+    if (rc < 0) return rc;
+  }
+  const LbaLayout &lay = L->lay;
   const int max_iter = 10;
   const size_t M_ub = std::min((size_t)w.W, E);
   LbaRef ref;
@@ -887,7 +666,7 @@
   bool delivered = false;
   L->seq = L->seq + 1 == 0 ? 1 : L->seq + 1;
   {
-    const int rc = lba_enqueue(s, w, maxn, M_ub, head, ref, t, n, max_iter, &res_dev, L->seq, &delivered);
+    const int rc = lba_enqueue(s, split, kfd, w, maxn, M_ub, head, ref, t, n, max_iter, &res_dev, L->seq, &delivered);
     if (rc < 0) return rc;
   }
   double *o_T = (double *)L->h_res, *o_e = o_T + 16 * LBA_KW;
```

Result: no change. 2729, median of 6 (+0.8%).
